# BIT-DYN/OpenObj

Hardware: AMD Instinct MI355X
Metric: training rays/sec/GPU @64 samples/ray, 50 obj; PSNR delta vs ref (higher is better)
Workload: dtype f32; 1 GPU; c2: Replica room_0-shaped, 50 object MLPs on this GPU (hidden 32), 4096 rays/object/step, 64 samples/ray (16+48), RGB+depth+opacity loss, fused fwd+loss+bwd+AdamW; objects_per_gpu=50, objects_total=50, rays_per_object=4096, samples_per_ray=64, hidden=32, feature_head=False, background_mlp=True, parallelism=objects sharded x1, rccl_ranks=1, launched_by=single process, loss_status=0

## Files before the change

include/objnerf_hip.h:

```cpp
#ifndef OBJNERF_HIP_H
#define OBJNERF_HIP_H

#include <stddef.h>
#include <stdint.h>

#ifdef __cplusplus
extern "C" {
#endif

#define OBJNERF_ABI_VERSION 14

#define OBJNERF_OK 0
#define OBJNERF_EINVAL (-22)
#define OBJNERF_ENOTSUP (-95)
#define OBJNERF_ELAUNCH (-5)

#define OBJNERF_N_TENSORS 19

enum objnerf_tensor {
  OBJNERF_T_IN_W = 0, OBJNERF_T_IN_B, OBJNERF_T_M1_W, OBJNERF_T_M1_B, OBJNERF_T_CAT_W,
  OBJNERF_T_CAT_B, OBJNERF_T_M2_W, OBJNERF_T_M2_B, OBJNERF_T_ALPHA_W, OBJNERF_T_ALPHA_B,
  OBJNERF_T_CL_W, OBJNERF_T_CL_B, OBJNERF_T_OC_W, OBJNERF_T_OC_B, OBJNERF_T_FL_W, OBJNERF_T_FL_B,
  OBJNERF_T_OF_W, OBJNERF_T_OF_B, OBJNERF_T_PE_B
};
// ... 46 lines not shown
  float box[4];
} objnerf_ingest_item;
int objnerf_ingest_frame(int32_t W, int32_t H, const uint8_t* rgb, const float* depth, const int32_t* inst,
                         const float* t_wc, int32_t K, const objnerf_ingest_item* items, void* stream);

int objnerf_box_rays(int64_t P, const float* T_WC, const float* T_OC, const float* half_extent,
                     const float* dirs_C, float* out_dirs_W, float* out_near, float* out_far,
                     uint8_t* out_hit, void* stream);
int objnerf_box_points(int64_t n, int32_t n_bins, const float* origin , const float* dirs_W,
                       const float* near, const float* far, const float* u, uint64_t seed, uint32_t draw,
                       float* out_z, float* out_pts, void* stream);

int objnerf_render_fwd(const objnerf_net* net, int64_t n, int32_t n_bins, const float* params, const float* scale,
                       const float* origin , const float* dirs_W, const float* near, const float* far,
                       const float* u, uint64_t seed, uint32_t draw, float* out_depth, float* out_opacity,
                       float* out_rgb, float* out_hfeat, float* out_z, int32_t mode, void* stream);

int objnerf_eval_points(const objnerf_net* net, int32_t K, int64_t N, const float* params,
                        int64_t p_stride, const float* scale, const float* pts, float* out_alpha,
                        float* out_color, float* out_hfeat, float* out_clip, void* stream);

size_t objnerf_eval_workspace_bytes(const objnerf_net* net, int32_t K, int64_t N);
int objnerf_eval_points_ws(const objnerf_net* net, int32_t K, int64_t N, const float* params,
                           int64_t p_stride, const float* scale, const float* pts, float* out_alpha,
                           float* out_color, float* out_hfeat, float* out_clip, void* workspace,
                           size_t workspace_bytes, void* stream);

int objnerf_mlp_forward(const objnerf_net* net, int32_t K, int64_t N, const float* params,
                        int64_t p_stride, const float* emb, float* out_alpha, float* out_color,
                        float* out_hfeat, float* out_clip, void* stream);

int objnerf_mlp_forward_ws(const objnerf_net* net, int32_t K, int64_t N, const float* params,
                           int64_t p_stride, const float* emb, float* out_alpha, float* out_color,
                           float* out_hfeat, float* out_clip, void* workspace, size_t workspace_bytes,
                           void* stream);

size_t objnerf_mlp_backward_workspace_bytes(const objnerf_net* net, int32_t K, int64_t N, int32_t with_clip);
int objnerf_mlp_backward_ws(const objnerf_net* net, int32_t K, int64_t N, const float* params,
                            int64_t p_stride, const float* emb, const float* d_alpha, const float* d_color,
                            const float* d_clip, float* grads, float* d_emb, void* workspace,
                            size_t workspace_bytes, void* stream);

int objnerf_embed_bwd(const objnerf_net* net, int32_t K, int64_t N, const float* params, int64_t p_stride,
                      const float* scale, const float* pts, const float* d_emb, float* d_B, float* scratch,
                      void* stream);

int objnerf_embed(const objnerf_net* net, int32_t K, int64_t N, const float* params,
                  int64_t p_stride, const float* scale, const float* pts, float* out_emb,
                  void* stream);

#define OBJNERF_COMPOSITE_INPUT_IS_OCCUPANCY 1
int objnerf_composite(int64_t n_rays, int32_t S, int32_t flags, const float* alpha, const float* color,
                      const float* z, const float* vals, int32_t V, float* out_term,
                      float* out_depth, float* out_var, float* out_rgb, float* out_opacity,
                      float* out_vals, void* stream);

int objnerf_mfma_peak(int32_t dtype, int32_t iters, int32_t n_wg, float* sink, void* stream);

int objnerf_occupancy(int64_t n, const float* alpha, float* out, void* stream);

int objnerf_feature_head(const objnerf_net* net, int32_t K, int64_t n, const float* params,
                         int64_t p_stride, const float* hfeat, const float* weight, float* out,
                         void* stream);

typedef struct objnerf_loss_args {
  int32_t K, R, S, C;
  float color_scaling, opacity_scaling, feat_scaling, reserved;
  const float* alpha; const float* color; const float* z; const float* gt_depth;
  const float* gt_rgb; const uint8_t* labels; const float* pred_feat; const float* gt_feat;
  const int32_t* flags_in;
  const int32_t* counts_in;
  float* loss_terms; float* total; float* d_alpha; float* d_color; float* d_pred_feat;
  int32_t* counts; int32_t* status;
} objnerf_loss_args;
int objnerf_step_batch_loss(const objnerf_loss_args* a, void* stream);

int objnerf_label_counts(int32_t K, int32_t R, const uint8_t* labels, int32_t* counts,
                         int32_t* flags_out, void* stream);

#define OBJNERF_TRAIN_BF16 1
#define OBJNERF_TRAIN_FP16 4
#define OBJNERF_TRAIN_LAYERWISE 2
#define OBJNERF_TRAIN_SELF_COUNTS 8
struct objnerf_context;
int objnerf_context_create(struct objnerf_context** out);
int objnerf_context_destroy(struct objnerf_context* ctx);

typedef struct objnerf_adamw_args {
  float* exp_avg; float* exp_avg_sq;
  int32_t* group_steps; int32_t bank; int32_t reserved;
  float lr, beta1, beta2, eps, weight_decay, reserved_f;
} objnerf_adamw_args;

typedef struct objnerf_train_args {
  int32_t K, R, S, mode;
  float color_scaling, opacity_scaling, feat_scaling, obj_center;
  const float* params; int64_t p_stride; const float* scale;
  const float* pts; const float* origins; const float* dirs; const float* z;
  const float* gt_depth; const float* gt_rgb; const uint8_t* labels; const float* gt_feat;
  const int32_t* counts; const int32_t* flags;
  float* grads; float* loss_terms; int32_t* status;
  void* workspace; size_t workspace_bytes;
  uint8_t* relu_masks;
  struct objnerf_context* context;
  float* emb_debug;
  const objnerf_adamw_args* optim;
} objnerf_train_args;
size_t objnerf_train_workspace_bytes(const objnerf_net* net, int32_t K, int32_t R, int32_t S,
                                     int32_t with_feat);
int objnerf_train_step(const objnerf_net* net, const objnerf_train_args* a, void* stream);

int objnerf_adamw_step(int32_t K, int64_t P, int64_t p_stride, float* params, const float* grads,
                       float* exp_avg, float* exp_avg_sq, const uint8_t* has_grad, int32_t step,
                       float lr, float beta1, float beta2, float eps, float weight_decay,
                       void* stream);

int objnerf_adamw_step_flags(int32_t K, int64_t P, int64_t p_stride, float* params, const float* grads, float* exp_avg,
                             float* exp_avg_sq, const uint8_t* has_grad, const int32_t* flags, int32_t* group_steps,
                             int32_t bank, int64_t colour_lo, int64_t feature_lo, int64_t feature_hi, float lr,
                             float beta1, float beta2, float eps, float weight_decay, void* stream);

int objnerf_render(int64_t n_rays, int32_t S, int32_t C, const float* termination, const float* vals, float* out,
                   void* stream);

int objnerf_render_loss(int64_t n, int32_t C, int32_t mode, int32_t normalise, const float* render, const float* gt,
                        float* out, void* stream);
int objnerf_reduce_batch_loss(int32_t K, int32_t R, const float* loss_mat, const float* var, const uint8_t* mask,
                              int32_t l2, int32_t avg, int32_t* counts_ws, float* out, int32_t* status, void* stream);
int objnerf_make_grid(int32_t dim, float lo, float hi, const float* scale, const float* transform, float* out,
                      void* stream);
int objnerf_ray_box(int64_t n, const float* origins, const float* dirs, const float* bmin, const float* bmax,
                    float* out_near, float* out_far, uint8_t* out_hit, void* stream);
int objnerf_dirs_w(int64_t F, int64_t P, const float* T_WC, const float* dirs_C, float* out_dirs_W, void* stream);
int objnerf_stratified_bins(int64_t n_rays, int32_t n_bins, const float* lo, float lo_scalar, const float* hi,
                            float hi_scalar, const float* u, uint64_t seed, uint64_t offset, float* out, void* stream);
int objnerf_normal_bins(int64_t n_rays, int32_t n_bins, const float* depth, float delta, const float* g, uint64_t seed,
                        uint64_t offset, float* out, void* stream);

#define OBJNERF_MC_DESCENT 1
size_t objnerf_mc_workspace_bytes(int32_t dim);
int objnerf_mc_count(int32_t dim, float level, const float* vol, void* ws, size_t ws_bytes, int64_t* out_counts,
                     void* stream);
int objnerf_mc_emit(int32_t dim, float level, int32_t flags, const float* vol, void* ws, size_t ws_bytes,
                    int64_t max_verts, int64_t max_faces, float* out_verts, float* out_normals, int32_t* out_faces,
                    void* stream);
int objnerf_mc_tables(uint8_t* edge_c0, uint8_t* edge_axis, uint8_t* ntri, uint8_t* tri);

typedef struct objnerf_voxel_args {
  int32_t K, F, W, H;
  double fx, fy, cx, cy, voxel;
  const objnerf_kf_store* table; const int32_t* n_keyframes; const double* camera_pose;
  const objnerf_kf_crops* crops;
} objnerf_voxel_args;
size_t objnerf_voxel_workspace_bytes(int32_t K, int32_t F, int32_t W, int32_t H);
int objnerf_voxel_scan(const objnerf_voxel_args* a, void* ws, size_t ws_bytes, int64_t* out_total, double* out_minmax,
                       void* stream);
int objnerf_voxel_emit(const objnerf_voxel_args* a, const void* ws, size_t ws_bytes, int32_t k0, int32_t k1,
                       const int64_t* base, const double* vmin, const int64_t* dims, int64_t n_points, double* out_pts,
                       int64_t* out_keys, void* stream);
size_t objnerf_voxel_heads_workspace_bytes(int64_t n);
int objnerf_voxel_heads(int64_t n, const int64_t* sorted_keys, int64_t* ws, void* stream);
int objnerf_voxel_centroids(int64_t n, const int64_t* sorted_keys, const int64_t* perm, const double* pts,
                            const int64_t* ws, int64_t max_voxels, double* out_centroids, int64_t* out_keys,
                            int64_t* out_first, void* stream);

typedef struct objnerf_obb_args {
  int32_t K, reserved;
  const double* verts; const int64_t* vert_off; const double* normals; const int32_t* edges; const int32_t* cand;
  const int64_t* cand_off; const int32_t* mode;
} objnerf_obb_args;
int objnerf_obb_search(const objnerf_obb_args* a, int32_t n_split, double* ws, double* out, void* stream);

#define OBJNERF_PROJ_COSINE 1
#define OBJNERF_PROJ_PER_SEGMENT 2
typedef struct objnerf_project_args {
  int32_t S, D, Q, flags;
  int64_t V, row_stride;
  const float* feat; const int64_t* seg_off; const float* W; const float* bias;
  float* out; float* minmax;
} objnerf_project_args;
size_t objnerf_project_workspace_bytes(int32_t S, int32_t Q, int64_t V);
int objnerf_project(const objnerf_project_args* a, void* ws, size_t ws_bytes, void* stream);

typedef struct objnerf_moments_args {
  int32_t S, D;
  int64_t V, row_stride;
  const float* feat; const int64_t* seg_off;
  double* mean; double* scatter;
} objnerf_moments_args;
size_t objnerf_moments_workspace_bytes(int32_t S, int32_t D);
int objnerf_moments(const objnerf_moments_args* a, void* ws, size_t ws_bytes, void* stream);

#define OBJNERF_COLOR_RGB 0
// ... 222 lines not shown
```

openobj_amd/_lib.py:

```python
from __future__ import annotations

import ctypes as C
import os
from typing import Optional

import torch

_HERE = os.path.dirname(os.path.abspath(__file__))
LIB_PATH = os.environ.get("OBJNERF_LIB") or os.path.join(_HERE, "csrc", "libobjnerf_hip.so")

OBJNERF_N_TENSORS = 19
ABI_VERSION = 14


class ObjnerfError(RuntimeError):
    pass


class Net(C.Structure):
    _fields_ = [("hidden", C.c_int32), ("feat_dim", C.c_int32), ("n_freqs", C.c_int32),
                ("reserved", C.c_int32)]


class SampleArgs(C.Structure):
    _fields_ = [("F", C.c_int32), ("W", C.c_int32), ("H", C.c_int32), ("n_frames", C.c_int32),
                ("n_px", C.c_int32), ("n_cam2surf", C.c_int32), ("n_bins", C.c_int32),
                ("obj_index", C.c_int32),
                ("surface_eps", C.c_float), ("stop_eps", C.c_float), ("min_bound", C.c_float),
                ("obj_center", C.c_float),
                ("rgbs", C.c_void_p), ("depth", C.c_void_p), ("t_wc", C.c_void_p), ("bbox", C.c_void_p),
                ("rays_dir_cache", C.c_void_p),
                ("kf_ids", C.c_void_p), ("u_w", C.c_void_p), ("u_h", C.c_void_p), ("u", C.c_void_p),
                ("g", C.c_void_p),
                ("out_rgb", C.c_void_p), ("out_depth", C.c_void_p), ("out_valid", C.c_void_p),
                ("out_labels", C.c_void_p), ("out_z", C.c_void_p), ("out_pts", C.c_void_p),
                ("max_depth_ws", C.c_void_p),
                ("seed", C.c_uint64), ("draw", C.c_uint32), ("reserved", C.c_uint32),
                ("kf_meta", C.c_void_p), ("out_kf", C.c_void_p), ("out_px", C.c_void_p),
                ("out_origins", C.c_void_p), ("out_dirs", C.c_void_p),
                ("global_partfeat", C.c_void_p), ("use_frame", C.c_void_p), ("out_partfeat", C.c_void_p),
                ("pf_frames", C.c_int32), ("pf_w", C.c_int32), ("pf_h", C.c_int32), ("pf_c", C.c_int32),
                ("pf_stride", C.c_int32), ("part_down", C.c_float),
                ("part_index", C.c_void_p), ("pf_rows", C.c_int32), ("reserved_pf", C.c_int32)]


class IngestItem(C.Structure):
    _fields_ = [("rgbs", C.c_void_p), ("depth", C.c_void_p), ("t_wc", C.c_void_p), ("bbox", C.c_void_p),
                ("slot", C.c_int32), ("obj_id", C.c_int32), ("box", C.c_float * 4)]


class LossArgs(C.Structure):
    _fields_ = [("K", C.c_int32), ("R", C.c_int32), ("S", C.c_int32), ("C", C.c_int32),
                ("color_scaling", C.c_float), ("opacity_scaling", C.c_float),
                ("feat_scaling", C.c_float), ("reserved", C.c_float),
                ("alpha", C.c_void_p), ("color", C.c_void_p), ("z", C.c_void_p), ("gt_depth", C.c_void_p),
                ("gt_rgb", C.c_void_p), ("labels", C.c_void_p), ("pred_feat", C.c_void_p),
                ("gt_feat", C.c_void_p), ("flags_in", C.c_void_p), ("counts_in", C.c_void_p),
                ("loss_terms", C.c_void_p), ("total", C.c_void_p), ("d_alpha", C.c_void_p),
                ("d_color", C.c_void_p), ("d_pred_feat", C.c_void_p),
                ("counts", C.c_void_p), ("status", C.c_void_p)]


TRAIN_BF16 = 1
TRAIN_SELF_COUNTS = 8


class AdamWArgs(C.Structure):
    _fields_ = [("exp_avg", C.c_void_p), ("exp_avg_sq", C.c_void_p), ("group_steps", C.c_void_p),
                ("bank", C.c_int32), ("reserved", C.c_int32),
                ("lr", C.c_float), ("beta1", C.c_float), ("beta2", C.c_float), ("eps", C.c_float),
                ("weight_decay", C.c_float), ("reserved_f", C.c_float)]


class TrainArgs(C.Structure):
    _fields_ = [("K", C.c_int32), ("R", C.c_int32), ("S", C.c_int32), ("mode", C.c_int32),
                ("color_scaling", C.c_float), ("opacity_scaling", C.c_float),
                ("feat_scaling", C.c_float), ("obj_center", C.c_float),
                ("params", C.c_void_p), ("p_stride", C.c_int64), ("scale", C.c_void_p),
                ("pts", C.c_void_p), ("origins", C.c_void_p), ("dirs", C.c_void_p), ("z", C.c_void_p),
                ("gt_depth", C.c_void_p), ("gt_rgb", C.c_void_p), ("labels", C.c_void_p),
                ("gt_feat", C.c_void_p),
                ("counts", C.c_void_p), ("flags", C.c_void_p),
                ("grads", C.c_void_p), ("loss_terms", C.c_void_p), ("status", C.c_void_p),
                ("workspace", C.c_void_p), ("workspace_bytes", C.c_size_t),
                ("relu_masks", C.c_void_p), ("context", C.c_void_p), ("emb_debug", C.c_void_p),
                ("optim", C.c_void_p)]


class KfStore(C.Structure):
    _fields_ = [("rgbs", C.c_void_p), ("depth", C.c_void_p), ("t_wc", C.c_void_p), ("bbox", C.c_void_p)]


class KfCrops(C.Structure):
    _fields_ = [("base", C.c_void_p), ("cap", C.c_int64), ("rect", C.c_void_p), ("t_wc", C.c_void_p),
                ("bbox", C.c_void_p)]


class IngestCropItem(C.Structure):
    _fields_ = [("store", KfCrops), ("slot", C.c_int32), ("obj_id", C.c_int32), ("box", C.c_float * 4),
                ("rect", C.c_int32 * 4)]


class VoxelArgs(C.Structure):
    _fields_ = [("K", C.c_int32), ("F", C.c_int32), ("W", C.c_int32), ("H", C.c_int32),
                ("fx", C.c_double), ("fy", C.c_double), ("cx", C.c_double), ("cy", C.c_double), ("voxel", C.c_double),
                ("table", C.c_void_p), ("n_keyframes", C.c_void_p), ("camera_pose", C.c_void_p),
                ("crops", C.c_void_p)]


class ObbArgs(C.Structure):
    _fields_ = [("K", C.c_int32), ("reserved", C.c_int32), ("verts", C.c_void_p), ("vert_off", C.c_void_p),
                ("normals", C.c_void_p), ("edges", C.c_void_p), ("cand", C.c_void_p), ("cand_off", C.c_void_p),
                ("mode", C.c_void_p)]


class ProjectArgs(C.Structure):
    _fields_ = [("S", C.c_int32), ("D", C.c_int32), ("Q", C.c_int32), ("flags", C.c_int32),
                ("V", C.c_int64), ("row_stride", C.c_int64),
                ("feat", C.c_void_p), ("seg_off", C.c_void_p), ("W", C.c_void_p), ("bias", C.c_void_p),
                ("out", C.c_void_p), ("minmax", C.c_void_p)]


class MomentsArgs(C.Structure):
    _fields_ = [("S", C.c_int32), ("D", C.c_int32), ("V", C.c_int64), ("row_stride", C.c_int64),
                ("feat", C.c_void_p), ("seg_off", C.c_void_p), ("mean", C.c_void_p), ("scatter", C.c_void_p)]


class ColorArgs(C.Structure):
    _fields_ = [("S", C.c_int32), ("Q", C.c_int32), ("V", C.c_int64), ("rgb_stride", C.c_int64),
                ("seg_off", C.c_void_p), ("mode", C.c_void_p), ("rgb", C.c_void_p), ("factor", C.c_void_p),
                ("constant", C.c_void_p), ("column", C.c_void_p), ("proj", C.c_void_p), ("minmax", C.c_void_p),
                ("out", C.c_void_p)]


class RayBoxesArgs(C.Structure):
    _fields_ = [("F", C.c_int32), ("N", C.c_int32), ("W", C.c_int32), ("H", C.c_int32),
                ("fx", C.c_double), ("fy", C.c_double), ("cx", C.c_double), ("cy", C.c_double),
                ("depth", C.c_void_p), ("twc", C.c_void_p), ("boxes", C.c_void_p), ("out", C.c_void_p)]


class MaskPointsArgs(C.Structure):
    _fields_ = [("n", C.c_int64), ("W", C.c_int32), ("H", C.c_int32),
                ("fx", C.c_double), ("fy", C.c_double), ("cx", C.c_double), ("cy", C.c_double),
                ("pix", C.c_void_p), ("depth", C.c_void_p), ("pose", C.c_void_p), ("out", C.c_void_p)]


class MapPointsHead(C.Structure):
# ... 5 lines not shown
    _fields_ = [("of_w", C.c_void_p), ("of_b", C.c_void_p), ("hfeat", C.c_void_p), ("row0", C.c_int64),
                ("n_rows", C.c_int64), ("H", C.c_int32), ("reserved", C.c_int32)]


class AffinityArgs(C.Structure):
    _fields_ = [("N", C.c_int32), ("F", C.c_int32), ("d_cap", C.c_int32), ("d_clip", C.c_int32),
                ("w_geo", C.c_double), ("w_cap", C.c_double), ("w_clip", C.c_double), ("w_color", C.c_double),
                ("w_geo2d", C.c_double),
                ("boxes", C.c_void_p), ("cap", C.c_void_p), ("clip", C.c_void_p), ("color", C.c_void_p),
                ("boxes2d", C.c_void_p), ("W", C.c_void_p), ("terms", C.c_void_p)]


PROJ_COSINE = 1
PROJ_PER_SEGMENT = 2
COLOR_RGB, COLOR_CONSTANT, COLOR_RAINBOW, COLOR_PCA = 0, 1, 2, 3


SIGNATURES = {
    "objnerf_abi_version": (C.c_int, []),
    "objnerf_context_create": (C.c_int, [C.POINTER(C.c_void_p)]),
    "objnerf_context_destroy": (C.c_int, [C.c_void_p]),
    "objnerf_param_layout": (C.c_int64, [C.POINTER(Net), C.POINTER(C.c_int64)]),
    "objnerf_rays_dirs": (C.c_int, [C.c_int32, C.c_int32, C.c_float, C.c_float, C.c_float, C.c_float,
                                    C.c_void_p, C.c_void_p]),
    "objnerf_sample_rays": (C.c_int, [C.POINTER(SampleArgs), C.c_void_p]),
    "objnerf_sample_rays_stacked": (C.c_int, [C.POINTER(SampleArgs), C.c_int32, C.c_void_p, C.c_void_p]),
    "objnerf_sample_points": (C.c_int, [C.POINTER(SampleArgs), C.c_void_p, C.c_void_p, C.c_void_p, C.c_void_p, C.c_void_p]),
    "objnerf_ingest_frame": (C.c_int, [C.c_int32, C.c_int32, C.c_void_p, C.c_void_p, C.c_void_p, C.c_void_p, C.c_int32,
                                       C.c_void_p, C.c_void_p]),
    "objnerf_box_rays": (C.c_int, [C.c_int64, C.c_void_p, C.c_void_p, C.c_void_p, C.c_void_p, C.c_void_p, C.c_void_p,
                                   C.c_void_p, C.c_void_p, C.c_void_p]),
    "objnerf_box_points": (C.c_int, [C.c_int64, C.c_int32, C.c_void_p, C.c_void_p, C.c_void_p, C.c_void_p, C.c_void_p,
                                     C.c_uint64, C.c_uint32, C.c_void_p, C.c_void_p, C.c_void_p]),
    "objnerf_render_fwd": (C.c_int, [C.POINTER(Net), C.c_int64, C.c_int32, C.c_void_p, C.c_void_p, C.c_void_p, C.c_void_p,
                                     C.c_void_p, C.c_void_p, C.c_void_p, C.c_uint64, C.c_uint32, C.c_void_p, C.c_void_p,
                                     C.c_void_p, C.c_void_p, C.c_void_p, C.c_int32, C.c_void_p]),
    "objnerf_eval_points": (C.c_int, [C.POINTER(Net), C.c_int32, C.c_int64, C.c_void_p, C.c_int64,
                                      C.c_void_p, C.c_void_p, C.c_void_p, C.c_void_p, C.c_void_p,
                                      C.c_void_p, C.c_void_p]),
    "objnerf_eval_workspace_bytes": (C.c_size_t, [C.POINTER(Net), C.c_int32, C.c_int64]),
    "objnerf_eval_points_ws": (C.c_int, [C.POINTER(Net), C.c_int32, C.c_int64, C.c_void_p, C.c_int64,
                                         C.c_void_p, C.c_void_p, C.c_void_p, C.c_void_p, C.c_void_p,
                                         C.c_void_p, C.c_void_p, C.c_size_t, C.c_void_p]),
    "objnerf_mlp_forward": (C.c_int, [C.POINTER(Net), C.c_int32, C.c_int64, C.c_void_p, C.c_int64,
                                      C.c_void_p, C.c_void_p, C.c_void_p, C.c_void_p, C.c_void_p,
                                      C.c_void_p]),
    "objnerf_mlp_forward_ws": (C.c_int, [C.POINTER(Net), C.c_int32, C.c_int64, C.c_void_p, C.c_int64,
                                         C.c_void_p, C.c_void_p, C.c_void_p, C.c_void_p, C.c_void_p,
                                         C.c_void_p, C.c_size_t, C.c_void_p]),
    "objnerf_embed": (C.c_int, [C.POINTER(Net), C.c_int32, C.c_int64, C.c_void_p, C.c_int64, C.c_void_p,
                                C.c_void_p, C.c_void_p, C.c_void_p]),
    "objnerf_mlp_backward_workspace_bytes": (C.c_size_t, [C.POINTER(Net), C.c_int32, C.c_int64, C.c_int32]),
    "objnerf_mlp_backward_ws": (C.c_int, [C.POINTER(Net), C.c_int32, C.c_int64, C.c_void_p, C.c_int64, C.c_void_p,
                                          C.c_void_p, C.c_void_p, C.c_void_p, C.c_void_p, C.c_void_p, C.c_void_p,
                                          C.c_size_t, C.c_void_p]),
    "objnerf_embed_bwd": (C.c_int, [C.POINTER(Net), C.c_int32, C.c_int64, C.c_void_p, C.c_int64, C.c_void_p, C.c_void_p,
                                    C.c_void_p, C.c_void_p, C.c_void_p, C.c_void_p]),
    "objnerf_occupancy": (C.c_int, [C.c_int64, C.c_void_p, C.c_void_p, C.c_void_p]),
    "objnerf_render": (C.c_int, [C.c_int64, C.c_int32, C.c_int32, C.c_void_p, C.c_void_p, C.c_void_p, C.c_void_p]),
    "objnerf_render_loss": (C.c_int, [C.c_int64, C.c_int32, C.c_int32, C.c_int32, C.c_void_p, C.c_void_p, C.c_void_p,
                                      C.c_void_p]),
    "objnerf_reduce_batch_loss": (C.c_int, [C.c_int32, C.c_int32, C.c_void_p, C.c_void_p, C.c_void_p, C.c_int32, C.c_int32,
                                            C.c_void_p, C.c_void_p, C.c_void_p, C.c_void_p]),
    "objnerf_make_grid": (C.c_int, [C.c_int32, C.c_float, C.c_float, C.c_void_p, C.c_void_p, C.c_void_p, C.c_void_p]),
    "objnerf_ray_box": (C.c_int, [C.c_int64, C.c_void_p, C.c_void_p, C.c_void_p, C.c_void_p, C.c_void_p, C.c_void_p,
                                  C.c_void_p, C.c_void_p]),
    "objnerf_dirs_w": (C.c_int, [C.c_int64, C.c_int64, C.c_void_p, C.c_void_p, C.c_void_p, C.c_void_p]),
    "objnerf_stratified_bins": (C.c_int, [C.c_int64, C.c_int32, C.c_void_p, C.c_float, C.c_void_p, C.c_float, C.c_void_p,
                                          C.c_uint64, C.c_uint64, C.c_void_p, C.c_void_p]),
    "objnerf_normal_bins": (C.c_int, [C.c_int64, C.c_int32, C.c_void_p, C.c_float, C.c_void_p, C.c_uint64, C.c_uint64,
                                      C.c_void_p, C.c_void_p]),
    "objnerf_mfma_peak": (C.c_int, [C.c_int32, C.c_int32, C.c_int32, C.c_void_p, C.c_void_p]),
    "objnerf_composite": (C.c_int, [C.c_int64, C.c_int32, C.c_int32, C.c_void_p, C.c_void_p, C.c_void_p, C.c_void_p,
                                    C.c_int32, C.c_void_p, C.c_void_p, C.c_void_p, C.c_void_p, C.c_void_p,
                                    C.c_void_p, C.c_void_p]),
    "objnerf_feature_head": (C.c_int, [C.POINTER(Net), C.c_int32, C.c_int64, C.c_void_p, C.c_int64,
                                       C.c_void_p, C.c_void_p, C.c_void_p, C.c_void_p]),
    "objnerf_step_batch_loss": (C.c_int, [C.POINTER(LossArgs), C.c_void_p]),
    "objnerf_label_counts": (C.c_int, [C.c_int32, C.c_int32, C.c_void_p, C.c_void_p, C.c_void_p,
                                       C.c_void_p]),
    "objnerf_train_workspace_bytes": (C.c_size_t, [C.POINTER(Net), C.c_int32, C.c_int32, C.c_int32,
                                                   C.c_int32]),
    "objnerf_train_step": (C.c_int, [C.POINTER(Net), C.POINTER(TrainArgs), C.c_void_p]),
    "objnerf_adamw_step": (C.c_int, [C.c_int32, C.c_int64, C.c_int64, C.c_void_p, C.c_void_p, C.c_void_p,
                                     C.c_void_p, C.c_void_p, C.c_int32, C.c_float, C.c_float, C.c_float,
                                     C.c_float, C.c_float, C.c_void_p]),
    "objnerf_adamw_step_flags": (C.c_int, [C.c_int32, C.c_int64, C.c_int64, C.c_void_p, C.c_void_p, C.c_void_p, C.c_void_p,
                                           C.c_void_p, C.c_void_p, C.c_void_p, C.c_int32, C.c_int64, C.c_int64, C.c_int64,
                                           C.c_float, C.c_float, C.c_float, C.c_float, C.c_float, C.c_void_p]),
    "objnerf_mc_workspace_bytes": (C.c_size_t, [C.c_int32]),
    "objnerf_mc_count": (C.c_int, [C.c_int32, C.c_float, C.c_void_p, C.c_void_p, C.c_size_t, C.c_void_p, C.c_void_p]),
    "objnerf_mc_emit": (C.c_int, [C.c_int32, C.c_float, C.c_int32, C.c_void_p, C.c_void_p, C.c_size_t, C.c_int64,
                                  C.c_int64, C.c_void_p, C.c_void_p, C.c_void_p, C.c_void_p]),
    "objnerf_mc_tables": (C.c_int, [C.c_void_p, C.c_void_p, C.c_void_p, C.c_void_p]),
    "objnerf_voxel_workspace_bytes": (C.c_size_t, [C.c_int32, C.c_int32, C.c_int32, C.c_int32]),
    "objnerf_voxel_scan": (C.c_int, [C.POINTER(VoxelArgs), C.c_void_p, C.c_size_t, C.c_void_p, C.c_void_p, C.c_void_p]),
    "objnerf_voxel_emit": (C.c_int, [C.POINTER(VoxelArgs), C.c_void_p, C.c_size_t, C.c_int32, C.c_int32, C.c_void_p,
                                     C.c_void_p, C.c_void_p, C.c_int64, C.c_void_p, C.c_void_p, C.c_void_p]),
    "objnerf_voxel_heads_workspace_bytes": (C.c_size_t, [C.c_int64]),
    "objnerf_voxel_heads": (C.c_int, [C.c_int64, C.c_void_p, C.c_void_p, C.c_void_p]),
    "objnerf_voxel_centroids": (C.c_int, [C.c_int64, C.c_void_p, C.c_void_p, C.c_void_p, C.c_void_p, C.c_int64,
                                          C.c_void_p, C.c_void_p, C.c_void_p, C.c_void_p]),
    "objnerf_obb_search": (C.c_int, [C.POINTER(ObbArgs), C.c_int32, C.c_void_p, C.c_void_p, C.c_void_p]),
    "objnerf_project_workspace_bytes": (C.c_size_t, [C.c_int32, C.c_int32, C.c_int64]),
    "objnerf_project": (C.c_int, [C.POINTER(ProjectArgs), C.c_void_p, C.c_size_t, C.c_void_p]),
    "objnerf_moments_workspace_bytes": (C.c_size_t, [C.c_int32, C.c_int32]),
    "objnerf_moments": (C.c_int, [C.POINTER(MomentsArgs), C.c_void_p, C.c_size_t, C.c_void_p]),
    "objnerf_vertex_colors": (C.c_int, [C.POINTER(ColorArgs), C.c_void_p]),
    "objnerf_rainbow_lut": (C.c_int, [C.c_void_p]),
    "objnerf_cell_keys": (C.c_int, [C.c_int64, C.c_int32, C.c_void_p, C.c_void_p, C.c_double, C.c_double, C.c_void_p,
                                    C.c_void_p, C.c_void_p, C.c_void_p]),
    "objnerf_dbscan_workspace_bytes": (C.c_size_t, [C.c_int64]),
    "objnerf_dbscan": (C.c_int, [C.c_int64, C.c_int32, C.c_void_p, C.c_void_p, C.c_void_p, C.c_void_p, C.c_void_p,
                                 C.c_double, C.c_void_p, C.c_size_t, C.c_void_p, C.c_void_p]),
    "objnerf_cloud_overlap": (C.c_int, [C.c_int64, C.c_int32, C.c_void_p, C.c_void_p, C.c_void_p, C.c_void_p, C.c_double,
                                        C.c_void_p, C.c_void_p]),
    "objnerf_mask_ray_boxes": (C.c_int, [C.POINTER(RayBoxesArgs), C.c_void_p]),
    "objnerf_mask_points": (C.c_int, [C.POINTER(MaskPointsArgs), C.c_void_p]),
    "objnerf_mask_hist": (C.c_int, [C.c_int64, C.c_int32, C.c_void_p, C.c_void_p, C.c_void_p, C.c_int32, C.c_int32,
                                    C.c_void_p, C.c_void_p]),
    "objnerf_point_bounds": (C.c_int, [C.c_int64, C.c_int32, C.c_void_p, C.c_void_p, C.c_void_p, C.c_void_p]),
    "objnerf_affinity_workspace_bytes": (C.c_size_t, [C.c_int32]),
    "objnerf_mask_affinity": (C.c_int, [C.POINTER(AffinityArgs), C.c_void_p, C.c_size_t, C.c_void_p, C.c_void_p]),
    "objnerf_mask_edges": (C.c_int, [C.c_int32, C.c_void_p, C.c_void_p, C.c_int64, C.c_void_p, C.c_void_p, C.c_void_p]),
    "objnerf_part_index": (C.c_int, [C.c_int32, C.c_int32, C.c_int32, C.c_void_p, C.c_void_p, C.c_void_p]),
    "objnerf_part_dense": (C.c_int, [C.c_int64, C.c_int32, C.c_int32, C.c_void_p, C.c_void_p, C.c_void_p, C.c_void_p]),
    "objnerf_ingest_frame_crops": (C.c_int, [C.c_int32, C.c_int32, C.c_void_p, C.c_void_p, C.c_void_p, C.c_void_p,
                                             C.c_int32, C.c_void_p, C.c_void_p, C.c_void_p]),
    "objnerf_sample_rays_crops": (C.c_int, [C.POINTER(SampleArgs), C.c_int32, C.c_void_p, C.c_void_p]),
    "objnerf_mappoints_workspace_bytes": (C.c_size_t, [C.c_int64, C.c_int32]),
    "objnerf_mappoints_count": (C.c_int, [C.c_int64, C.c_int32, C.c_void_p, C.c_void_p, C.c_void_p, C.c_size_t, C.c_void_p,
                                          C.c_void_p]),
    "objnerf_mappoints_emit": (C.c_int, [C.c_int64, C.c_int32, C.c_void_p, C.c_void_p, C.c_void_p, C.c_size_t, C.c_int64,
                                         C.c_void_p, C.c_void_p]),
    "objnerf_mappoints_eval": (C.c_int, [C.POINTER(Net), C.c_int32, C.c_int64, C.c_int64, C.c_void_p, C.c_int64, C.c_void_p,
                                         C.c_void_p, C.c_void_p, C.c_void_p, C.c_void_p, C.c_void_p, C.c_void_p, C.c_void_p,
                                         C.c_void_p, C.c_void_p, C.c_void_p]),
    "objnerf_mappoints_gather": (C.c_int, [C.c_int64, C.c_void_p, C.c_void_p, C.c_float, C.c_void_p, C.c_void_p]),
    "objnerf_mappoints_merge": (C.c_int, [C.c_int64, C.c_int64, C.c_void_p, C.c_void_p, C.c_int32, C.c_void_p, C.c_void_p]),
    "objnerf_mappoints_resolve": (C.c_int, [C.c_int64, C.c_int32, C.c_int64, C.c_void_p, C.c_void_p, C.c_void_p, C.c_void_p, C.c_void_p,
                                            C.c_void_p, C.c_void_p, C.c_void_p]),
    "objnerf_mappoints_head_workspace_bytes": (C.c_size_t, [C.c_int64]),
    "objnerf_mappoints_head": (C.c_int, [C.c_int32, C.c_int32, C.c_int64, C.c_int64, C.c_void_p, C.c_void_p, C.c_void_p,
                                         C.c_void_p, C.c_int32, C.c_void_p, C.c_size_t, C.c_void_p, C.c_void_p, C.c_void_p]),
    "objnerf_mesh_sample_workspace_bytes": (C.c_size_t, [C.c_int64, C.c_int32]),
    "objnerf_mesh_sample": (C.c_int, [C.c_int64, C.c_int64, C.c_int32, C.c_int64, C.c_void_p, C.c_void_p, C.c_void_p,
                                      C.c_void_p, C.c_uint64, C.c_void_p, C.c_size_t, C.c_void_p, C.c_void_p, C.c_void_p,
                                      C.c_void_p]),
    "objnerf_nearest_workspace_bytes": (C.c_size_t, [C.c_int64, C.c_int32]),
    "objnerf_nearest": (C.c_int, [C.c_int64, C.c_int64, C.c_int32, C.c_void_p, C.c_void_p, C.c_void_p, C.c_void_p,
                                  C.c_void_p, C.c_double, C.c_void_p, C.c_void_p, C.c_int32, C.c_void_p, C.c_size_t,
                                  C.c_void_p, C.c_void_p, C.c_void_p, C.c_void_p]),
    "objnerf_seg_stats": (C.c_int, [C.c_int64, C.c_int32, C.c_void_p, C.c_void_p, C.c_int32, C.POINTER(C.c_double),
                                    C.c_void_p, C.c_void_p]),
    "objnerf_vertex_views": (C.c_int, [C.c_int64, C.c_int32, C.c_int32, C.c_int32, C.c_void_p, C.c_void_p, C.c_void_p,
                                       C.c_double, C.c_double, C.c_double, C.c_double, C.c_double, C.c_double, C.c_int32,
                                       C.c_void_p, C.c_void_p]),
    "objnerf_mesh_cull_workspace_bytes": (C.c_size_t, [C.c_int64, C.c_int64]),
    "objnerf_mesh_cull_count": (C.c_int, [C.c_int64, C.c_int64, C.c_int32, C.c_void_p, C.c_void_p, C.c_void_p, C.c_size_t,
                                          C.c_void_p, C.c_void_p, C.c_void_p]),
    "objnerf_mesh_cull_emit": (C.c_int, [C.c_int64, C.c_int64, C.c_int32, C.c_void_p, C.c_void_p, C.c_void_p, C.c_size_t,
                                         C.c_int64, C.c_int64, C.c_void_p, C.c_void_p, C.c_void_p, C.c_void_p, C.c_void_p]),
    "objnerf_view_rays_workspace_bytes": (C.c_size_t, [C.c_int64, C.c_int32]),
    "objnerf_view_rays_count": (C.c_int, [C.c_int64, C.c_int32, C.c_void_p, C.c_void_p, C.c_void_p, C.c_void_p, C.c_size_t,
                                          C.c_void_p, C.c_void_p]),
    "objnerf_view_rays_emit": (C.c_int, [C.c_int64, C.c_int32, C.c_void_p, C.c_void_p, C.c_void_p, C.c_void_p, C.c_size_t,
# ... 102 lines not shown
```

openobj_amd/csrc/objnerf_generic.h:

```cpp
#pragma once
#include "../../include/objnerf_hip.h"
namespace objmisc {
struct LossHoisted {
  int Hh;
  const float* hf; const float* rayin; const float* gram;
  float* d_hf; float* rayfeat;
};
int step_batch_loss_impl(const objnerf_loss_args* a, const LossHoisted* hz, void* stream, float* loss_part);
int adamw_flags_range(int32_t K, int64_t P, int64_t p_stride, float* params, const float* grads, float* exp_avg,
                      float* exp_avg_sq, const uint8_t* has_grad, const int32_t* flags, int32_t* group_steps, int32_t bank,
                      int64_t colour_lo, int64_t feature_lo, int64_t feature_hi, int64_t ng_lo, int64_t ng_hi, float lr,
                      float beta1, float beta2, float eps, float weight_decay, void* stream);
int label_counts_only(int32_t K, int32_t R, const uint8_t* labels, int32_t* counts, void* stream);
}

namespace objgen {
size_t train_workspace_bytes(const objnerf_net* net, int K, int R, int S, int feat, int sixteen = 0);
int train_step(const objnerf_net* net, const objnerf_train_args* a, void* stream, int* done = nullptr);
struct Operand { const float* p; long s0, s1, bs; bool h16; };
inline Operand op_rows(const float* p, long ld, long bs, bool h16 = false) { return {p, ld, 1, bs, h16}; }
inline Operand op_cols(const float* p, long ld, long bs, bool h16 = false) { return {p, 1, ld, bs, h16}; }
struct FeatHeadArgs { int K, R, Hh, C; const float* P; long ps; int off_w, off_b; const float* gt_feat; };
void feat_gram(void* stream, const FeatHeadArgs& h, float* gram, long gstride);
void feature_head(void* stream, const FeatHeadArgs& h, long n, const float* hfeat, const float* weight, float* out);
void gemm_f32(void* stream, int batch, int M, int N, int Kd, const Operand& A, const Operand& B, const Operand& C,
              bool accumulate);
size_t wgrad_parts_floats(int batch, int M, int N, long n);
void wgrad_f32(void* stream, int batch, int M, int N, long n, const Operand& A, const Operand& B, const Operand& C,
               float* parts, size_t parts_floats);
struct FeatHead {
  float *gram, *rayin, *rayfeat, *X1, *X2, *Tm, *mom, *parts; size_t parts_floats;
};
size_t feat_head_workspace_bytes(int K, int R, int Hh, int C);
FeatHead feat_head_carve(char* base, int K, int R, int Hh, int C);
int feat_head_prep(void* stream, const FeatHeadArgs& h, const FeatHead& f, int operands);
int feat_head_grads(void* stream, const FeatHeadArgs& h, const FeatHead& f, float* grads, int operands);
size_t eval_workspace_bytes(const objnerf_net* net, int K, long N);
int eval_points(const objnerf_net* net, int K, long N, const float* params, long p_stride, const float* scale,
                const float* pts, float* out_alpha, float* out_color, float* out_hfeat, float* out_clip,
                void* workspace, size_t workspace_bytes, void* stream, const float* emb_in = nullptr);
size_t mlp_backward_workspace_bytes(const objnerf_net* net, int K, long N, int with_clip);
int mlp_backward(const objnerf_net* net, int K, long N, const float* params, long p_stride, const float* emb,
                 const float* d_alpha, const float* d_color, const float* d_clip, float* grads, float* d_emb,
                 void* workspace, size_t workspace_bytes, void* stream);
int embed_backward(const objnerf_net* net, int K, long N, const float* params, long p_stride, const float* scale,
                   const float* pts, const float* d_emb, float* d_B, float* scratch, void* stream);
}

namespace obj256 {
bool applicable(const objnerf_net* net, const objnerf_train_args* a);
size_t workspace_bytes(int K, int R, int S, int feat = 0, int C = 0);
int train_step(const objnerf_net* net, const objnerf_train_args* a, void* stream);
}
```

openobj_amd/csrc/objnerf_misc.hip:

```cpp
#include "objnerf_device.h"
#include "objnerf_philox.h"
#include "objnerf_wg.h"
#include "objnerf_generic.h"
#include "objnerf_step_tail.h"
#include "objnerf_boxray.h"

namespace {

__device__ __forceinline__ float sgnf(float x) { return x > 0.f ? 1.0f : (x < 0.f ? -1.0f : 0.0f); }

__global__ __launch_bounds__(256) void composite_kernel(long n_rays, int S, int in_is_occ, const float* alpha,
                                                        const float* color, const float* z, const float* vals,
                                                        int V, float* out_term,
                                                        float* out_depth, float* out_var, float* out_rgb,
                                                        float* out_opacity, float* out_vals) {
  extern __shared__ float sm[];
  const int lane = threadIdx.x & 63, w = threadIdx.x >> 6;
  float* wv = sm + (long)w * S;
  const long ray = (long)blockIdx.x * 4 + w;
  if (ray >= n_rays) return;
  float carry = 1.0f, D = 0.f, O = 0.f, C0 = 0.f, C1 = 0.f, C2 = 0.f;
  for (int s0 = 0; s0 < S; s0 += 64) {
    const int s = s0 + lane;
    const bool on = s < S;
    const float al = on ? alpha[ray * S + s] : 0.f;
    const float occ = on ? (in_is_occ ? al : sigmoid_acc(al)) : 0.f;
    const float fr = on ? (1.0f - occ) + 1e-10f : 1.0f;
    const float pinc = SegRows::make(64, lane).scan_mul(fr, lane) * carry;
    float T = __shfl_up(pinc, 1, 64);
    if (lane == 0) T = carry;
    carry = __shfl(pinc, 63, 64);
    const float wt = occ * T;
    if (on) {
      wv[s] = wt;
      if (out_term) out_term[ray * S + s] = wt;
    }
    const float zz = (on && z) ? z[ray * S + s] : 0.f;
    D += wave_sum64(wt * zz);
    O += wave_sum64(wt);
    if (color) {
      const float* cp = color + (ray * S + s) * 3;
      C0 += wave_sum64(on ? wt * cp[0] : 0.f);
      C1 += wave_sum64(on ? wt * cp[1] : 0.f);
      C2 += wave_sum64(on ? wt * cp[2] : 0.f);
    }
  }
  float Vv = 0.f;
  for (int s0 = 0; s0 < S; s0 += 64) {
    const int s = s0 + lane;
    const bool on = s < S;
    const float dz = (on && z) ? z[ray * S + s] - D : 0.f;
    Vv += wave_sum64(on ? wv[s] * (dz * dz) : 0.f);
  }
  if (lane == 0) {
    if (out_depth) out_depth[ray] = D;
    if (out_var) out_var[ray] = Vv;
    if (out_opacity) out_opacity[ray] = O;
    if (out_rgb) { out_rgb[ray * 3] = C0; out_rgb[ray * 3 + 1] = C1; out_rgb[ray * 3 + 2] = C2; }
  }
  if (vals && out_vals) {
    for (int v = lane; v < V; v += 64) {
      float acc = 0.f;
      for (int s = 0; s < S; ++s) acc += wv[s] * vals[(ray * S + s) * (long)V + v];
      out_vals[ray * (long)V + v] = acc;
    }
  }
}


__global__ void embed_kernel(int K, long N, int n_freqs, const float* params, long p_stride, long off_B,
                             const float* scale, const float* pts, float* out) {
  const int E = 3 + OBJ_NDIR * n_freqs;
  const long idx = (long)blockIdx.x * blockDim.x + threadIdx.x;
  const int k = blockIdx.y;
  if (idx >= N * E) return;
  const long i = idx / E;
  const int e = (int)(idx - i * E);
  const float* B = params + (long)k * p_stride + off_B;
  const float sc = scale[k];
  const float* p = pts + ((long)k * N + i) * 3;
  float v;
  if (e < 3) {
    v = p[e] / sc;
  } else {
    const float t0 = p[0] / sc, t1 = p[1] / sc, t2 = p[2] / sc;
    const int f = (e - 3) / OBJ_NDIR, j = (e - 3) - f * OBJ_NDIR;
    const float pj = fmaf(t2, B[3 * j + 2], fmaf(t1, B[3 * j + 1], t0 * B[3 * j]));
    v = sin_acc((pj * (float)(1 << f)) * OBJ_PI_F);
  }
  out[(long)k * N * E + idx] = v;
}

__global__ void occupancy_kernel(long n, const float* alpha, float* out) {
  const long i = (long)blockIdx.x * blockDim.x + threadIdx.x;
  if (i < n) out[i] = sigmoid_acc(alpha[i]);
}

__global__ void label_counts_kernel(int K, int R, const uint8_t* labels, int* counts, int* flags) {
  const int k = blockIdx.x;
  int c1 = 0, c2 = 0;
  for (int r = threadIdx.x; r < R; r += blockDim.x) {
    const int l = labels[(long)k * R + r];
    c1 += (l == 1);
    c2 += (l != 2);
  }
  __shared__ int s1[4], s2[4];
  for (int d = 32; d >= 1; d >>= 1) {
    c1 += __shfl_xor(c1, d, 64);
    c2 += __shfl_xor(c2, d, 64);
  }
  if ((threadIdx.x & 63) == 0) { s1[threadIdx.x >> 6] = c1; s2[threadIdx.x >> 6] = c2; }
  __syncthreads();
  if (threadIdx.x == 0) {
    const int a = s1[0] + s1[1] + s1[2] + s1[3], b = s2[0] + s2[1] + s2[2] + s2[3];
    counts[2 * k] = a;
    counts[2 * k + 1] = b;
    if (!flags) return;
    if (K == 1) {
      flags[0] = a == 0;
      flags[1] = b == 0;
    } else {
      if (a == 0) atomicOr(&flags[0], 1);
      if (b == 0) atomicOr(&flags[1], 1);
    }
  }
}

__global__ void loss_prologue_kernel(int K, const int* counts_in, int* counts, int* flags, const int* flags_in,
                                     float* loss_terms) {
  __shared__ int f[2];
  if (threadIdx.x < 2) f[threadIdx.x] = (flags_in && flags_in[threadIdx.x]) ? 1 : 0;
  __syncthreads();
  for (int k = threadIdx.x; k < K; k += blockDim.x) {
    const int a = counts_in[2 * k], b = counts_in[2 * k + 1];
    counts[2 * k] = a;
    counts[2 * k + 1] = b;
    if (a == 0) atomicOr(&f[0], 1);
    if (b == 0) atomicOr(&f[1], 1);
  }
  for (int i = threadIdx.x; i < 4 * K; i += blockDim.x) loss_terms[i] = 0.f;
  __syncthreads();
  if (threadIdx.x < 2) flags[threadIdx.x] = f[threadIdx.x];
}

__global__ void merge_flags_kernel(int* flags, const int* flags_in) {
  if (threadIdx.x < 2 && flags_in && flags_in[threadIdx.x]) flags[threadIdx.x] = 1;
}

struct LossDev {
  int K, R, S, C;
  float cs, os, fs;
  const float* alpha; const float* color; const float* z; const float* gt_depth; const float* gt_rgb;
  const uint8_t* labels; const float* pred_feat; const float* gt_feat;
  const int* counts; const int* flags;
  float* loss_terms; float* d_alpha; float* d_color; float* d_pred_feat;
  int Hh;
  const float* hf;
  const float* rayin;
  const float* gram;
  float* d_hf;
  float* rayfeat;
  float* loss_part;
};

__global__ __launch_bounds__(1024) void loss_kernel(const LossDev a) {
  extern __shared__ float sm[];
  __shared__ float s_red[16][4];
  const int lane = threadIdx.x & 63, w = threadIdx.x >> 6;
  const int nw = blockDim.x >> 6;
  const int S = a.S;
  float* wv = sm + (long)w * (3 * S + 2 * a.Hh);
  float* tv = wv + S;
  float* dwv = tv + S;
  float* sfh = dwv + S;
  float* sgf = sfh + a.Hh;
  const long rr = (long)blockIdx.x * nw + w;
  const int k = (int)(rr / a.R);
  const float n1 = (float)a.counts[2 * k], n2 = (float)a.counts[2 * k + 1];
  const float inv1 = a.flags[0] ? 0.0f : 1.0f / (n1 + 1e-10f);
  const float inv2 = a.flags[1] ? 0.0f : 1.0f / (n2 + 1e-10f);
  const int lab = a.labels[rr];
  const float m1 = (lab == 1) ? 1.f : 0.f, m2 = (lab != 2) ? 1.f : 0.f, tgt = (lab != 0) ? 1.f : 0.f;
  float carry = 1.0f, D = 0.f, O = 0.f, C0 = 0.f, C1 = 0.f, C2 = 0.f;
  for (int s0 = 0; s0 < S; s0 += 64) {
    const int s = s0 + lane;
    const bool on = s < S;
    const float occ = on ? sigmoid_acc(a.alpha[rr * S + s]) : 0.f;
    const float fr = on ? (1.0f - occ) + 1e-10f : 1.0f;
    const float pinc = SegRows::make(64, lane).scan_mul(fr, lane) * carry;
    float T = __shfl_up(pinc, 1, 64);
    if (lane == 0) T = carry;
    carry = __shfl(pinc, 63, 64);
    const float wt = occ * T;
    if (on) { wv[s] = wt; tv[s] = T; dwv[s] = 0.f; }
    const float* cp = a.color + (rr * S + (on ? s : 0)) * 3;
    D += wave_sum64(on ? wt * a.z[rr * S + s] : 0.f);
    O += wave_sum64(wt);
    C0 += wave_sum64(on ? wt * cp[0] : 0.f);
    C1 += wave_sum64(on ? wt * cp[1] : 0.f);
    C2 += wave_sum64(on ? wt * cp[2] : 0.f);
  }
  float Vv = 0.f;
  for (int s0 = 0; s0 < S; s0 += 64) {
    const int s = s0 + lane;
    const bool on = s < S;
    const float dz = on ? a.z[rr * S + s] - D : 0.f;
// ... 494 lines not shown
  const float* o = origins_ws + (long)i * 3;
  const float* dr = dirs_ws + (long)i * 3;
  for (int s = 0; s < S; ++s) {
    float* p = a.out_pts + ((long)i * S + s) * 3;
    p[0] = (o[0] + dr[0] * z[s]) - a.obj_center;
    p[1] = (o[1] + dr[1] * z[s]) - a.obj_center;
    p[2] = (o[2] + dr[2] * z[s]) - a.obj_center;
  }
}

__global__ void sample_prepare_kernel(const objnerf_sample_args a, const uint8_t* __restrict__ rgbs4,
                                      const float* __restrict__ depth, const float* __restrict__ origins,
                                      const float* __restrict__ dirs_w, float* origins_ws, float* dirs_ws) {
  const int i = blockIdx.x * blockDim.x + threadIdx.x;
  const int n = a.n_frames * a.n_px;
  if (i >= n) return;
  const uint8_t* px = rgbs4 + (long)i * 4;
  a.out_rgb[i * 3] = px[0]; a.out_rgb[i * 3 + 1] = px[1]; a.out_rgb[i * 3 + 2] = px[2];
  a.out_labels[i] = px[3];
  const float d = depth[i];
  a.out_depth[i] = d;
  atomicMax((int*)a.max_depth_ws, __float_as_int(fmaxf(d, 0.0f)));
  const int f = i / a.n_px;
#pragma unroll
  for (int r = 0; r < 3; ++r) {
    origins_ws[i * 3 + r] = origins[f * 3 + r];
    dirs_ws[i * 3 + r] = dirs_w[i * 3 + r];
  }
}

}

#define CLEAR_STALE() (void)hipGetLastError()

namespace objmisc {
int step_batch_loss_impl(const objnerf_loss_args* a, const LossHoisted* hz, void* stream, float* loss_part) {
  CLEAR_STALE();
  if (!a || !a->alpha || !a->color || !a->z || !a->gt_depth || !a->gt_rgb || !a->labels || !a->loss_terms ||
      !a->counts || a->K <= 0 || a->R <= 0 || a->S <= 0)
    return OBJNERF_EINVAL;
  if (!hz && (a->pred_feat == nullptr) != (a->gt_feat == nullptr)) return OBJNERF_EINVAL;
  if (hz && (!a->gt_feat || a->pred_feat || !hz->hf || !hz->rayin || !hz->gram || !hz->d_hf || !hz->rayfeat || hz->Hh <= 0))
    return OBJNERF_EINVAL;
  if (a->S > 2048) return OBJNERF_ENOTSUP;
  hipStream_t st = (hipStream_t)stream;
  int* flags = a->counts + 2 * a->K;
  if (a->counts_in) {
    hipLaunchKernelGGL(loss_prologue_kernel, dim3(1), dim3(256), 0, st, a->K, a->counts_in, a->counts, flags, a->flags_in,
                       a->loss_terms);
  } else {
    if (a->K > 1) (void)hipMemsetAsync(flags, 0, 2 * sizeof(int), st);
    hipLaunchKernelGGL(label_counts_kernel, dim3(a->K), dim3(256), 0, st, a->K, a->R, a->labels, a->counts, flags);
    if (a->flags_in) hipLaunchKernelGGL(merge_flags_kernel, dim3(1), dim3(64), 0, st, flags, a->flags_in);
    (void)hipMemsetAsync(a->loss_terms, 0, (size_t)a->K * 4 * sizeof(float), st);
  }
  LossDev d;
  d.K = a->K; d.R = a->R; d.S = a->S; d.C = a->C;
  d.cs = a->color_scaling; d.os = a->opacity_scaling; d.fs = a->feat_scaling;
  d.alpha = a->alpha; d.color = a->color; d.z = a->z; d.gt_depth = a->gt_depth; d.gt_rgb = a->gt_rgb;
  d.labels = a->labels; d.pred_feat = a->pred_feat; d.gt_feat = a->gt_feat; d.counts = a->counts; d.flags = flags;
  d.loss_terms = a->loss_terms; d.d_alpha = a->d_alpha; d.d_color = a->d_color; d.d_pred_feat = a->d_pred_feat;
  d.Hh = hz ? hz->Hh : 0;
  d.hf = hz ? hz->hf : nullptr; d.rayin = hz ? hz->rayin : nullptr; d.gram = hz ? hz->gram : nullptr;
  d.d_hf = hz ? hz->d_hf : nullptr; d.rayfeat = hz ? hz->rayfeat : nullptr;
  const long nr = (long)a->K * a->R;
  int rb = 16;
  while (rb > 1 && (a->R % rb != 0 || (size_t)rb * (3 * a->S + 2 * d.Hh) * 4 > 60000)) rb >>= 1;
  d.loss_part = loss_part;
  hipLaunchKernelGGL(loss_kernel, dim3((unsigned)(nr / rb)), dim3(64 * rb), (size_t)rb * (3 * a->S + 2 * d.Hh) * 4, st, d);
  CHECK_LAUNCH();
  hipLaunchKernelGGL(loss_total_kernel, dim3(1), dim3(256), 0, st, a->K, a->loss_terms, a->color_scaling,
                     a->opacity_scaling, (a->pred_feat || hz) ? a->feat_scaling : 0.0f, a->total, a->status,
                     (const float*)loss_part, a->R / rb);
  CHECK_LAUNCH();
  return OBJNERF_OK;
}
int label_counts_only(int32_t K, int32_t R, const uint8_t* labels, int32_t* counts, void* stream) {
  CLEAR_STALE();
  if (K <= 0 || R <= 0 || !labels || !counts) return OBJNERF_EINVAL;
  hipLaunchKernelGGL(label_counts_kernel, dim3(K), dim3(256), 0, (hipStream_t)stream, K, R, labels, counts, (int*)nullptr);
  CHECK_LAUNCH();
  return OBJNERF_OK;
}
int adamw_flags_range(int32_t K, int64_t P, int64_t p_stride, float* params, const float* grads, float* exp_avg,
                      float* exp_avg_sq, const uint8_t* has_grad, const int32_t* flags, int32_t* group_steps, int32_t bank,
                      int64_t colour_lo, int64_t feature_lo, int64_t feature_hi, int64_t ng_lo, int64_t ng_hi, float lr,
                      float beta1, float beta2, float eps, float weight_decay, void* stream) {
  CLEAR_STALE();
  if (K <= 0 || P <= 0 || p_stride < P || !params || !grads || !exp_avg || !exp_avg_sq || !flags || !group_steps ||
      (bank != 0 && bank != 1) ||
      colour_lo > feature_lo || feature_lo > feature_hi || feature_hi > P)
    return OBJNERF_EINVAL;
  dim3 grid((unsigned)((P + 255) / 256), (unsigned)K);
  hipLaunchKernelGGL(adamw_dyn_kernel, grid, dim3(256), 0, (hipStream_t)stream, (long)P, (long)p_stride, params, grads,
                     exp_avg, exp_avg_sq, has_grad, flags, group_steps, (int)bank, (long)colour_lo, (long)feature_lo,
                     (long)feature_hi, (double)lr, (double)beta1, (double)beta2, eps, (double)weight_decay, (long)ng_lo,
                     (long)ng_hi);
  CHECK_LAUNCH();
  return OBJNERF_OK;
}
}

template <int DT>
__global__ __launch_bounds__(256) void mfma_peak_kernel(int iters, float* sink) {
  typedef float f16v __attribute__((ext_vector_type(16)));
  typedef __bf16 bf8 __attribute__((ext_vector_type(8)));
  const int lane = threadIdx.x & 63;
  f16v a0, a1;
  for (int i = 0; i < 16; ++i) { a0[i] = 0.f; a1[i] = 0.f; }
  const float av = 0.37f + 0.011f * lane, bv = -0.52f + 0.007f * (lane ^ 21);
  bf8 ab, bb;
  for (int i = 0; i < 8; ++i) { ab[i] = (__bf16)(av + 0.05f * i); bb[i] = (__bf16)(bv - 0.03f * i); }
  for (int i = 0; i < iters; ++i) {
    if (DT == 0) {
      a0 = __builtin_amdgcn_mfma_f32_32x32x2f32(av, bv, a0, 0, 0, 0);
      a1 = __builtin_amdgcn_mfma_f32_32x32x2f32(bv, av, a1, 0, 0, 0);
      a0 = __builtin_amdgcn_mfma_f32_32x32x2f32(av, av, a0, 0, 0, 0);
      a1 = __builtin_amdgcn_mfma_f32_32x32x2f32(bv, bv, a1, 0, 0, 0);
    } else {
      a0 = __builtin_amdgcn_mfma_f32_32x32x16_bf16(ab, bb, a0, 0, 0, 0);
      a1 = __builtin_amdgcn_mfma_f32_32x32x16_bf16(bb, ab, a1, 0, 0, 0);
      a0 = __builtin_amdgcn_mfma_f32_32x32x16_bf16(ab, ab, a0, 0, 0, 0);
      a1 = __builtin_amdgcn_mfma_f32_32x32x16_bf16(bb, bb, a1, 0, 0, 0);
    }
    if ((i & 127) == 127) { a0 *= 1e-3f; a1 *= 1e-3f; }
  }
  float r = 0.f;
  for (int i = 0; i < 16; ++i) r += a0[i] + a1[i];
  sink[blockIdx.x * 256 + threadIdx.x] = r;
}

extern "C" {

int objnerf_composite(int64_t n_rays, int32_t S, int32_t flags, const float* alpha, const float* color,
                      const float* z, const float* vals, int32_t V, float* out_term, float* out_depth, float* out_var,
                      float* out_rgb, float* out_opacity, float* out_vals, void* stream) {
  CLEAR_STALE();
  if (n_rays <= 0 || S <= 0 || !alpha) return OBJNERF_EINVAL;
  if (!z && (out_depth || out_var)) return OBJNERF_EINVAL;
  if (S > 4096) return OBJNERF_ENOTSUP;
  hipLaunchKernelGGL(composite_kernel, dim3((unsigned)((n_rays + 3) / 4)), dim3(256), (size_t)4 * S * 4,
                     (hipStream_t)stream, (long)n_rays, S, (int)(flags & OBJNERF_COMPOSITE_INPUT_IS_OCCUPANCY), alpha,
                     color, z, vals, V, out_term, out_depth, out_var, out_rgb, out_opacity, out_vals);
  CHECK_LAUNCH();
  return OBJNERF_OK;
}

int objnerf_mfma_peak(int32_t dtype, int32_t iters, int32_t n_wg, float* sink, void* stream) {
  CLEAR_STALE();
  if (!sink || iters <= 0 || n_wg <= 0 || (dtype != 0 && dtype != 1)) return OBJNERF_EINVAL;
  if (dtype == 0) hipLaunchKernelGGL(mfma_peak_kernel<0>, dim3(n_wg), dim3(256), 0, (hipStream_t)stream, iters, sink);
  else hipLaunchKernelGGL(mfma_peak_kernel<1>, dim3(n_wg), dim3(256), 0, (hipStream_t)stream, iters, sink);
  CHECK_LAUNCH();
  return OBJNERF_OK;
}

int objnerf_occupancy(int64_t n, const float* alpha, float* out, void* stream) {
  CLEAR_STALE();
  if (n <= 0 || !alpha || !out) return OBJNERF_EINVAL;
  hipLaunchKernelGGL(occupancy_kernel, dim3((unsigned)((n + 255) / 256)), dim3(256), 0, (hipStream_t)stream, (long)n,
                     alpha, out);
  CHECK_LAUNCH();
  return OBJNERF_OK;
}

int objnerf_feature_head(const objnerf_net* net, int32_t K, int64_t n, const float* params, int64_t p_stride,
// ... 207 lines not shown
```

openobj_amd/csrc/objnerf_train.hip:

```cpp
#include <mutex>
#include "objnerf_mlp32.h"
#include "objnerf_train_common.h"
#include "objnerf_generic.h"
#include "objnerf_wg.h"
#include "objnerf_step_tail.h"

using namespace obj32;
using namespace objtrain;

namespace {

struct EvalDev {
  int K, G; long N;
  const float* params; long p_stride; const float* scale; const float* pts; const float* emb;
  float* alpha; float* color; float* hfeat;
  Layout L;
};

constexpr int XCOLS = 33;
struct FinalizeArgs {
  const float* slab; const float* loss_part;
  int K, G; long P, slab_stride, p_stride;
  long ng_lo, ng_hi, ext_lo, ext_hi;
  float* grads; float* loss_terms; int* status;
  int flat_nwg, NT, Gs;
  float* params; float* m; float* v; const int* flags; int* steps; int bank;
  long lo1, lo2, hi2;
  double lr, b1, b2, wd; float eps;
  const int* counts_in; int* flags_out;
  const float* Tpart; const float* Mpart; const float* head_w; int Gfin, C; long of_w, of_b;
};
constexpr int FIN_EPT = 4;
__global__ __launch_bounds__(256) void finalize_kernel(const FinalizeArgs a) {
  const int k = blockIdx.y;
  const long i0 = (long)blockIdx.x * (256 * FIN_EPT) + threadIdx.x;
  __shared__ float s_step_size[3], s_bc2_sqrt[3];
  __shared__ int s_active[3];
  __shared__ int s_bad;
  __shared__ float s_M[XCOLS * XCOLS];
  const bool first = blockIdx.x == 0 && blockIdx.y == 0;
  if (a.counts_in && first && threadIdx.x == 64) {
    int e0, e1;
    early_flags_of_counts(a.counts_in, a.K, e0, e1);
    a.flags_out[0] = e0; a.flags_out[1] = e1;
  }
  if (a.params && threadIdx.x < 3) {
    const int g = threadIdx.x;
    int e0, e1;
    if (a.counts_in) early_flags_of_counts(a.counts_in, a.K, e0, e1);
    else { e0 = a.flags[0]; e1 = a.flags[1]; }
    adamw_group_begin(g, e0 != 0, e1 != 0, a.steps, a.bank, a.lr, a.b1, a.b2, first, s_active[g], s_step_size[g],
                      s_bc2_sqrt[g]);
  }
  if (first && threadIdx.x == 0) s_bad = 0;
  const long blk_lo = (long)blockIdx.x * (256 * FIN_EPT), blk_hi = blk_lo + 256 * FIN_EPT;
  const bool head_blk = a.Tpart && blk_lo < a.ext_hi && blk_hi > a.ext_lo;
  if (head_blk)
    for (int e = threadIdx.x; e < XCOLS * XCOLS; e += 256) {
      float v = 0.f;
      for (int g = 0; g < a.Gfin; ++g) v += a.Mpart[((long)k * a.Gfin + g) * XCOLS * XCOLS + e];
      s_M[e] = v;
    }
  if (a.params || first || head_blk) __syncthreads();
  int G = a.G;
  if (a.flat_nwg) {
    const long T = (long)a.K * a.NT;
    G = flat_wg_of(T, a.flat_nwg, (long)(k + 1) * a.NT - 1) - flat_wg_of(T, a.flat_nwg, (long)k * a.NT) + 1;
  }
  const int stride = a.flat_nwg ? a.Gs : a.G;
  float s[FIN_EPT];
  bool live[FIN_EPT], slabbed[FIN_EPT];
#pragma unroll
  for (int e = 0; e < FIN_EPT; ++e) {
    const long i = i0 + 256 * e;
    live[e] = i < a.P && !(i >= a.ng_lo && i < a.ng_hi);
    slabbed[e] = live[e] && !(i >= a.ext_lo && i < a.ext_hi);
    s[e] = 0.f;
  }
  const float* sl0 = a.slab + (long)k * stride * a.slab_stride + i0;
  for (int g = 0; g < G; ++g) {
    float t[FIN_EPT];
#pragma unroll
    for (int e = 0; e < FIN_EPT; ++e) t[e] = slabbed[e] ? sl0[(long)g * a.slab_stride + 256 * e] : 0.f;
#pragma unroll
    for (int e = 0; e < FIN_EPT; ++e) s[e] += t[e];
  }
#pragma unroll
  for (int e = 0; e < FIN_EPT; ++e) {
    const long i = i0 + 256 * e;
    if (!live[e]) continue;
    const long idx = (long)k * a.p_stride + i;
    float sv_ = s[e];
    if (!slabbed[e]) {
      if (a.Tpart) {
        const bool is_b = i >= a.of_b;
        const int cc = is_b ? (int)(i - a.of_b) : (int)((i - a.of_w) >> 5), hh = is_b ? 32 : (int)((i - a.of_w) & 31);
        const float* hw = a.head_w + (long)k * ((long)a.C * 33);
        const float* W = hw + cc * 32;
        const float bc = hw[a.C * 32 + cc];
        float v = 0.f;
        for (int g = 0; g < a.Gfin; ++g) v += a.Tpart[((long)k * a.Gfin + g) * a.C * XCOLS + cc * XCOLS + hh];
        if (!is_b) {
          for (int j = 0; j < 32; ++j) v = fmaf(W[j], s_M[j * XCOLS + hh], v);
          sv_ = fmaf(bc, s_M[32 * XCOLS + hh], v);
        } else {
          for (int j = 0; j < 32; ++j) v = fmaf(W[j], s_M[32 * XCOLS + j], v);
          sv_ = fmaf(bc, s_M[32 * XCOLS + 32], v);
        }
      } else {
        sv_ = a.grads[idx];
      }
    }
    s[e] = sv_;
  }
#pragma unroll
  for (int e = 0; e < FIN_EPT; ++e) {
    const long i = i0 + 256 * e;
    if (!live[e]) continue;
    const long idx = (long)k * a.p_stride + i;
    const float sv_ = s[e];
    if (slabbed[e] || a.Tpart) a.grads[idx] = sv_;
    if (a.params) {
      const int g = adamw_group_of(i, a.lo1, a.lo2, a.hi2);
      if (s_active[g]) {
        float decay, w1, beta2, w2;
        adamw_coeffs(a.lr, a.b1, a.b2, a.wd, decay, w1, beta2, w2);
        adamw_update(a.params, a.m, a.v, idx, sv_, decay, w1, beta2, w2, s_step_size[g], s_bc2_sqrt[g], a.eps);
      }
    }
  }
  if (first) {
    int bad = 0;
    for (int e = threadIdx.x; e < 4 * a.K; e += blockDim.x) {
      const int kk = e >> 2;
      int Gk = a.G;
      if (a.flat_nwg) {
        const long T = (long)a.K * a.NT;
        Gk = flat_wg_of(T, a.flat_nwg, (long)(kk + 1) * a.NT - 1) - flat_wg_of(T, a.flat_nwg, (long)kk * a.NT) + 1;
      }
      float sl = 0.f;
      for (int g = 0; g < Gk; ++g) sl += a.loss_part[((long)kk * stride + g) * 4 + (e & 3)];
      a.loss_terms[e] = sl;
      bad |= loss_status_bits(sl);
    }
    if (bad) atomicOr(&s_bad, bad);
    __syncthreads();
    if (threadIdx.x == 0) *a.status = s_bad;
  }
}

template <bool FEAT, bool FROM_EMB>
__global__ __launch_bounds__(256) void eval_kernel(const EvalDev a) {
  using namespace obj32n;
  extern __shared__ __attribute__((aligned(16))) float lds[];
  const int tid = threadIdx.x, lane = tid & 63;
  const int w = __builtin_amdgcn_readfirstlane(tid >> 6);
  const int c = lane & 15, g = lane >> 4;
  const int k = blockIdx.x / a.G, gi = blockIdx.x % a.G;
  stage_weights32(lds, a.params + (long)k * a.p_stride, a.L, FEAT, tid, 256);
  const float* sv = lds + sv_base(FEAT);
  const float* wf = (const float*)__builtin_assume_aligned(lds + 4 * g * WROW + out_pos(c), 8);
  const float scale = FROM_EMB ? 1.0f : a.scale[k];
  const long ntiles = (a.N + 63) / 64;
  for (long tile = gi; tile < ntiles; tile += a.G) {
    asm volatile("" ::: "memory");
    const long n = tile * 64 + 16 * w + c;
    const bool valid = n < a.N;
    const long o = (long)k * a.N + (valid ? n : 0);
    Emb32 e;
    if (FROM_EMB) {
      embed32_load(e, a.emb + o * OBJ_EMB, g);
    } else {
      const float* p = a.pts + o * 3;
      Pe32 pe;
      pe32_project(sv, g, p[0], p[1], p[2], scale, pe);
      embed32(e, pe, g);
    }
    Acts act;
    const float hout = mlp32_forward<FEAT>(wf, sv, g, e, act);
    if (valid) {
      if (g == 0) a.alpha[o] = hout;
      else a.color[o * 3 + g - 1] = hout;
      if (FEAT) {
#pragma unroll
        for (int tt = 0; tt < 2; ++tt) {
          float4 v = make_float4(act.hf.t[tt][0], act.hf.t[tt][1], act.hf.t[tt][2], act.hf.t[tt][3]);
          *reinterpret_cast<float4*>(a.hfeat + o * H + 16 * tt + 4 * g) = v;
        }
      }
    }
  }
}

__global__ __launch_bounds__(256) void feat_rowstats_kernel(const float* params, long p_stride, int off_b, int C, int R,
                                                            const float* gt_feat, float* rayin) {
  const int k = blockIdx.y;
  const int l16 = threadIdx.x & 15;
  const long r = (long)blockIdx.x * 16 + (threadIdx.x >> 4);
  const float* B = params + (long)k * p_stride + off_b;
  float bs = 0.f, gs = 0.f;
  if (r < R) {
    const float* gp = gt_feat + ((long)k * R + r) * C;
    for (int cc = 4 * l16; cc < C; cc += 64) {
      const float4 gv = *reinterpret_cast<const float4*>(gp + cc);
      bs = fmaf(B[cc + 3], gv.w, fmaf(B[cc + 2], gv.z, fmaf(B[cc + 1], gv.y, fmaf(B[cc], gv.x, bs))));
      gs = fmaf(gv.w, gv.w, fmaf(gv.z, gv.z, fmaf(gv.y, gv.y, fmaf(gv.x, gv.x, gs))));
    }
  }
  bs = dpp_rowsum16(bs);
  gs = dpp_rowsum16(gs);
  if (r < R && l16 == 0) {
    float* o = rayin + ((long)k * R + r) * RAYIN;
    o[32] = bs;
    o[33] = sqrtf(gs);
  }
}
constexpr int FEAT_PRE_MAXC = 512;
__global__ __launch_bounds__(512, 4) void feat_pre_kernel(const float* __restrict__ params, long p_stride, int off_w, int off_b,
                                                       int C, int R, const float* __restrict__ gt_feat,
                                                       float* __restrict__ rayin, float* __restrict__ gram,
                                                       float* __restrict__ head_snap, const uint8_t* __restrict__ labels,
                                                       int* __restrict__ counts) {
  extern __shared__ __attribute__((aligned(16))) float fp_lds[];
  const int k = blockIdx.y, tid = threadIdx.x, lane = tid & 63, w = tid >> 6;
// ... 272 lines not shown
                const float* scale, const float* pts, const float* emb, float* out_alpha, float* out_color,
                float* out_hfeat, float* out_clip, void* stream) {
  EvalDev d;
  d.K = K; d.N = N; d.params = params; d.p_stride = p_stride; d.scale = scale; d.pts = pts; d.emb = emb;
  d.alpha = out_alpha; d.color = out_color; d.hfeat = out_hfeat;
  d.L = make_layout(net->feat_dim);
  const long ntiles = (N + 63) / 64;
  long G = (2L * objnerf_num_cu()) / K;
  if (G < 1) G = 1;
  if (G > ntiles) G = ntiles;
  d.G = (int)G;
  hipStream_t st = (hipStream_t)stream;
  const bool feat = out_hfeat != nullptr;
  const size_t lds_bytes = (size_t)obj32n::img_floats(feat) * 4;
  objnerf_once_per_device([] {
    (void)hipFuncSetAttribute((const void*)eval_kernel<true, true>, hipFuncAttributeMaxDynamicSharedMemorySize,
                              obj32n::img_floats(true) * 4);
    (void)hipFuncSetAttribute((const void*)eval_kernel<true, false>, hipFuncAttributeMaxDynamicSharedMemorySize,
                              obj32n::img_floats(true) * 4);
  });
  const dim3 grid(K * d.G), blk(256);
  if (emb) {
    if (feat) hipLaunchKernelGGL((eval_kernel<true, true>), grid, blk, lds_bytes, st, d);
    else hipLaunchKernelGGL((eval_kernel<false, true>), grid, blk, lds_bytes, st, d);
  } else {
    if (feat) hipLaunchKernelGGL((eval_kernel<true, false>), grid, blk, lds_bytes, st, d);
    else hipLaunchKernelGGL((eval_kernel<false, false>), grid, blk, lds_bytes, st, d);
  }
  if (hipGetLastError() != hipSuccess) return OBJNERF_ELAUNCH;
  if (out_clip) return objnerf_feature_head(net, K, N, params, p_stride, out_hfeat, nullptr, out_clip, stream);
  return OBJNERF_OK;
}

}

extern "C" {

int objnerf_abi_version(void) { return OBJNERF_ABI_VERSION; }

int64_t objnerf_param_layout(const objnerf_net* net, int64_t offsets[OBJNERF_N_TENSORS + 1]) {
  if (!net || !offsets || net->hidden <= 0 || net->feat_dim <= 0) return OBJNERF_EINVAL;
  const int64_t H_ = net->hidden, C = net->feat_dim;
  const int64_t sizes[OBJNERF_N_TENSORS] = {H_ * OBJ_E1, H_, H_ * H_, H_, H_ * (H_ + OBJ_E1), H_, H_ * H_, H_, H_, 1,
                                            H_ * (H_ + OBJ_E2), H_, 3 * H_, 3, H_ * (H_ + OBJ_E2), H_, C * H_, C,
                                            OBJ_NDIR * 3};
  int64_t o = 0;
  for (int i = 0; i < OBJNERF_N_TENSORS; ++i) { offsets[i] = o; o += sizes[i]; }
  offsets[OBJNERF_N_TENSORS] = o;
  return (o + 63) / 64 * 64;
}

static int grid_cap(int K) {
  const int g = objnerf_num_cu() / (K > 0 ? K : 1);
  return g > 32 ? g : 32;
}
static int train_grid(int K, int NT) {
  constexpr long TILE_EQUIV = 4;
  const int cu = objnerf_num_cu();
  int gmax = grid_cap(K);
  if (gmax > NT) gmax = NT;
  if (gmax < 1) gmax = 1;
  int best = 1;
  long best_cost = -1;
  for (int G = 1; G <= gmax; ++G) {
    const long rounds = ((long)K * G + cu - 1) / cu;
    const long cost = rounds * ((NT + G - 1) / G + TILE_EQUIV);
    if (best_cost < 0 || cost < best_cost) { best = G; best_cost = cost; }
  }
  return best;
}

static void choose_flat(TrainDev& d, int K, const long TILE_EQUIV) {
  const int cu = objnerf_num_cu();
  const long T = (long)K * d.NT;
  if (T < cu) return;
  const long share = (T + cu - 1) / cu;
  const long segs = 1 + (share + d.NT - 1) / d.NT;
  const long cost_flat = share + segs * TILE_EQUIV;
  const long rounds = ((long)K * d.G + cu - 1) / cu;
  const long cost_strided = rounds * ((d.NT + d.G - 1) / d.G + TILE_EQUIV);
  const long gs = ((long)d.NT * cu + T - 1) / T + 1;
  if (cost_flat < cost_strided && gs <= grid_cap(K)) { d.flat_nwg = cu; d.Gs = (int)gs; }
}

struct Workspace32 {
  float* slab;
  float* loss_part;
  float *rayin, *gram, *rayfeat;
  float *X1, *X2;
  float *Tm, *mom;
  float *parts_t, *parts_m;
  float* head_snap;
  size_t bytes;
};
static Workspace32 workspace32(uintptr_t base, int K, int R, int C, int64_t ps, bool feat) {
  Workspace32 w = {};
  auto take = [&](size_t floats) { float* p = (float*)(base + w.bytes); w.bytes += align256(floats * 4); return p; };
  w.slab = take((size_t)K * grid_cap(K) * ps);
  w.loss_part = take((size_t)K * grid_cap(K) * 4);
  if (feat) {
    w.rayin = take((size_t)K * R * RAYIN);
    w.gram = take((size_t)K * GRAM);
    w.rayfeat = take((size_t)K * R * RAYFEAT);
    w.X1 = take((size_t)K * R * XCOLS);
    w.X2 = take((size_t)K * R * XCOLS);
    w.Tm = take((size_t)K * C * XCOLS + (size_t)K * XCOLS * XCOLS);
    w.mom = w.Tm + (size_t)K * C * XCOLS;
    w.parts_t = take(objgen::wgrad_parts_floats(K, C, XCOLS, R));
    w.parts_m = take(objgen::wgrad_parts_floats(K, XCOLS, XCOLS, R));
    w.head_snap = take((size_t)K * C * XCOLS);
  }
  return w;
}

size_t objnerf_train_workspace_bytes(const objnerf_net* net, int32_t K, int32_t R, int32_t S, int32_t with_feat) {
  if (!net || K <= 0 || R <= 0 || S <= 0) return 0;
  if (net->hidden != 32 || S > 64 || (with_feat & 2)) return objgen::train_workspace_bytes(net, K, R, S, with_feat & 1, (with_feat & 4) != 0);
  int64_t offs[OBJNERF_N_TENSORS + 1];
  const int64_t ps = objnerf_param_layout(net, offs);
  return workspace32(0, K, R, net->feat_dim, ps, (with_feat & 1) != 0).bytes;
}

int objnerf_train_step(const objnerf_net* net, const objnerf_train_args* a, void* stream) {
  (void)hipGetLastError();
  if (!net || !a || !a->params || !a->scale || !a->z || !a->gt_depth || !a->gt_rgb || !a->labels || !a->counts ||
      !a->flags || !a->grads || !a->loss_terms || !a->status || !a->workspace)
    return OBJNERF_EINVAL;
  if (!a->pts && (!a->origins || !a->dirs)) return OBJNERF_EINVAL;
  if (a->K <= 0 || a->R <= 0 || a->S <= 0) return OBJNERF_EINVAL;
  if (net->n_freqs != 6) return OBJNERF_ENOTSUP;
  if ((a->mode & OBJNERF_TRAIN_FP16) && (a->mode & OBJNERF_TRAIN_BF16)) return OBJNERF_EINVAL;
  if (a->optim && (!a->optim->exp_avg || !a->optim->exp_avg_sq || !a->optim->group_steps ||
                   (a->optim->bank != 0 && a->optim->bank != 1)))
    return OBJNERF_EINVAL;
  if (net->hidden != 32 || a->S > 64 || (a->mode & (OBJNERF_TRAIN_LAYERWISE | OBJNERF_TRAIN_FP16))) {
    if (a->workspace_bytes < objgen::train_workspace_bytes(net, a->K, a->R, a->S, a->gt_feat != nullptr,
                                                           (a->mode & (OBJNERF_TRAIN_FP16 | OBJNERF_TRAIN_BF16)) != 0))
      return OBJNERF_EINVAL;
    if (a->emb_debug) return OBJNERF_ENOTSUP;
    int done = 0;
    int rc;
#ifndef OBJ_NO_TRAIN256
    if (!(a->mode & OBJNERF_TRAIN_LAYERWISE) && obj256::applicable(net, a)) {
      if (a->mode & OBJNERF_TRAIN_SELF_COUNTS) {
        rc = objnerf_label_counts(a->K, a->R, a->labels, const_cast<int32_t*>(a->counts), const_cast<int32_t*>(a->flags), stream);
        if (rc) return rc;
      }
      rc = obj256::train_step(net, a, stream);
    } else
#endif
    rc = objgen::train_step(net, a, stream, &done);
    if (rc) return rc;
    if (a->optim && !(done & 2)) {
      int64_t offs[OBJNERF_N_TENSORS + 1];
      objnerf_param_layout(net, offs);
      const bool feat_ = a->gt_feat != nullptr;
      const objnerf_adamw_args* o = a->optim;
      return objmisc::adamw_flags_range(a->K, offs[OBJNERF_N_TENSORS], a->p_stride, const_cast<float*>(a->params), a->grads,
                                        o->exp_avg, o->exp_avg_sq, nullptr, a->flags, o->group_steps, o->bank,
                                        offs[OBJNERF_T_CL_W], offs[OBJNERF_T_FL_W], offs[OBJNERF_T_PE_B],
                                        feat_ ? offs[OBJNERF_N_TENSORS] : offs[OBJNERF_T_FL_W],
                                        feat_ ? offs[OBJNERF_N_TENSORS] : offs[OBJNERF_T_PE_B], o->lr, o->beta1, o->beta2,
                                        o->eps, o->weight_decay, stream);
    }
    return OBJNERF_OK;
  }
  const bool self_counts = (a->mode & OBJNERF_TRAIN_SELF_COUNTS) != 0;
  const bool feat = a->gt_feat != nullptr;
  const bool counts_in_pre = self_counts && feat && net->feat_dim <= FEAT_PRE_MAXC && net->feat_dim % 16 == 0;
  if (self_counts && !counts_in_pre) {
    const int rc = objmisc::label_counts_only(a->K, a->R, a->labels, const_cast<int32_t*>(a->counts), stream);
    if (rc) return rc;
  }
  if (feat && (TS / a->S) > 16) return OBJNERF_ENOTSUP;
  const bool bf16 = (a->mode & OBJNERF_TRAIN_BF16) != 0;
  if (bf16 && (a->relu_masks || a->emb_debug)) return OBJNERF_ENOTSUP;
  int64_t offs[OBJNERF_N_TENSORS + 1];
  const int64_t ps = objnerf_param_layout(net, offs);
  if (a->p_stride < offs[OBJNERF_N_TENSORS]) return OBJNERF_EINVAL;
  const int C = net->feat_dim;
  const Workspace32 ws = workspace32((uintptr_t)a->workspace, a->K, a->R, C, ps, feat);
  if (a->workspace_bytes < ws.bytes) return OBJNERF_EINVAL;

  TrainDev d;
  d.K = a->K; d.R = a->R; d.S = a->S;
  d.TR = TS / a->S;
  d.NT = (a->R + d.TR - 1) / d.TR;
  d.G = train_grid(a->K, d.NT);
  d.flat_nwg = 0; d.Gs = 0;
  d.color_scaling = a->color_scaling; d.opacity_scaling = a->opacity_scaling; d.feat_scaling = a->feat_scaling;
  d.obj_center = a->obj_center;
  d.params = a->params; d.p_stride = a->p_stride; d.scale = a->scale;
  d.pts = a->pts; d.origins = a->origins; d.dirs = a->dirs; d.z = a->z;
  d.gt_depth = a->gt_depth; d.gt_rgb = a->gt_rgb; d.labels = a->labels; d.gt_feat = a->gt_feat;
  d.counts = a->counts; d.flags = a->flags; d.derive_flags = self_counts ? 1 : 0;
  d.L = make_layout(net->feat_dim);
  d.slab = ws.slab;
  d.slab_stride = ps;
  d.loss_part = ws.loss_part;
  d.rayin = ws.rayin; d.gram = ws.gram; d.rayfeat = ws.rayfeat;
  d.relu_masks = a->relu_masks;
  d.emb_debug = a->emb_debug;

  hipStream_t st = (hipStream_t)stream;
  const float *fin_T = nullptr, *fin_M = nullptr;
  int fin_G = 0;
  if (feat) {
    const bool pre_one = C <= FEAT_PRE_MAXC && C % 16 == 0;
    if (!pre_one) objgen::feat_gram(stream, {a->K, 0, 32, C, a->params, (long)a->p_stride, d.L.of_w, d.L.of_b, nullptr}, ws.gram, GRAM);
    if (pre_one) {
      const size_t pre_lds = ((size_t)(C / 16) * 2 * 64 * 4 + C) * sizeof(float);
      objnerf_once_per_device([] {
        (void)hipFuncSetAttribute((const void*)feat_pre_kernel, hipFuncAttributeMaxDynamicSharedMemorySize,
                                  (int)(((FEAT_PRE_MAXC / 16) * 2 * 64 * 4 + FEAT_PRE_MAXC) * sizeof(float)));
      });
      int gpo = 2 * objnerf_num_cu() / a->K;
      if (gpo < 1) gpo = 1;
      if (gpo > (a->R + 127) / 128) gpo = (a->R + 127) / 128;
      hipLaunchKernelGGL(feat_pre_kernel, dim3(gpo, a->K), dim3(512), pre_lds, st, a->params, (long)a->p_stride,
                         d.L.of_w, d.L.of_b, C, a->R, a->gt_feat, ws.rayin, ws.gram, ws.head_snap, a->labels,
                         counts_in_pre ? const_cast<int32_t*>(a->counts) : nullptr);
    } else {
      objgen::gemm_f32(stream, a->K, a->R, 32, C, objgen::op_rows(a->gt_feat, C, (long)a->R * C),
                       objgen::op_rows(a->params + d.L.of_w, 32, (long)a->p_stride),
                       objgen::op_rows(ws.rayin, RAYIN, (long)a->R * RAYIN), false);
      hipLaunchKernelGGL(feat_rowstats_kernel, dim3((a->R + 15) / 16, a->K), dim3(256), 0, st, a->params,
                         (long)a->p_stride, d.L.of_b, C, a->R, a->gt_feat, ws.rayin);
    }
    if (bf16) launch_train_bf16(d, stream, true);
    else { choose_flat(d, a->K, 4); launch_train32(d, stream, true); }
    if (hipGetLastError() != hipSuccess) return OBJNERF_ELAUNCH;
    const long nr = (long)a->K * a->R;
    int gpo = 2 * objnerf_num_cu() / a->K;
    if (gpo < 1) gpo = 1;
    if (gpo > 16) gpo = 16;
    const size_t part_room = ((size_t)((char*)ws.X2 - (char*)ws.X1) / 4 + (size_t)a->K * a->R * XCOLS) / (size_t)a->K;
    while (gpo > 1 && (size_t)gpo * ((size_t)C * XCOLS + XCOLS * XCOLS) > part_room) --gpo;
    const bool one_pass = C == 512 && (size_t)gpo * ((size_t)C * XCOLS + XCOLS * XCOLS) <= part_room;
    int Gfin = 1;
    const float *Tsrc = ws.Tm, *Msrc = ws.mom;
    if (one_pass) {
      float* Tpart = ws.X1;
      float* Mpart = ws.X1 + (size_t)a->K * gpo * C * XCOLS;
      hipLaunchKernelGGL(feat_post_kernel, dim3(gpo, a->K), dim3(512), 0, st, C, a->R, a->gt_feat, ws.rayfeat, Tpart, Mpart);
      Gfin = gpo; Tsrc = Tpart; Msrc = Mpart;
    } else {
      hipLaunchKernelGGL(feat_scale_kernel, dim3((unsigned)((nr * XCOLS + 255) / 256)), dim3(256), 0, st, nr, ws.rayfeat, ws.X1, ws.X2);
      (void)hipMemsetAsync(ws.Tm, 0, ((size_t)a->K * C * XCOLS + (size_t)a->K * XCOLS * XCOLS) * 4, st);
      objgen::wgrad_f32(stream, a->K, C, XCOLS, a->R, objgen::op_cols(a->gt_feat, C, (long)a->R * C),
                        objgen::op_rows(ws.X1, XCOLS, (long)a->R * XCOLS), objgen::op_rows(ws.Tm, XCOLS, (long)C * XCOLS),
                        ws.parts_t, objgen::wgrad_parts_floats(a->K, C, XCOLS, a->R));
      objgen::wgrad_f32(stream, a->K, XCOLS, XCOLS, a->R, objgen::op_cols(ws.X2, XCOLS, (long)a->R * XCOLS),
                        objgen::op_rows(ws.rayfeat, RAYFEAT, (long)a->R * RAYFEAT),
                        objgen::op_rows(ws.mom, XCOLS, (long)XCOLS * XCOLS), ws.parts_m,
                        objgen::wgrad_parts_floats(a->K, XCOLS, XCOLS, a->R));
    }
    if (one_pass && pre_one) {
      fin_T = Tsrc; fin_M = Msrc; fin_G = Gfin;
    } else {
      hipLaunchKernelGGL(feat_finish_kernel, dim3((C * XCOLS + 255) / 256, a->K), dim3(256), 0, st, a->params,
                         (long)a->p_stride, d.L.of_w, d.L.of_b, C, Tsrc, Msrc, a->grads, Gfin);
    }
  } else if (bf16) {
    launch_train_bf16(d, stream, false);
  } else {
    choose_flat(d, a->K, 4);
    launch_train32(d, stream, false);
  }
  if (hipGetLastError() != hipSuccess) return OBJNERF_ELAUNCH;
  const long P = offs[OBJNERF_N_TENSORS];
  dim3 fg((unsigned)((P + 256 * FIN_EPT - 1) / (256 * FIN_EPT)), (unsigned)a->K);
  FinalizeArgs fa;
  fa.slab = d.slab; fa.loss_part = d.loss_part; fa.K = a->K; fa.G = d.G; fa.P = P; fa.slab_stride = (long)ps;
  fa.p_stride = (long)a->p_stride;
  fa.ng_lo = feat ? P : d.L.fl_w; fa.ng_hi = feat ? P : d.L.pe_b;
  fa.ext_lo = feat ? d.L.of_w : P; fa.ext_hi = feat ? d.L.pe_b : P;
  fa.grads = a->grads; fa.loss_terms = a->loss_terms; fa.status = a->status;
  fa.flat_nwg = d.flat_nwg; fa.NT = d.NT; fa.Gs = d.Gs;
  fa.params = nullptr; fa.m = fa.v = nullptr; fa.flags = a->flags; fa.steps = nullptr; fa.bank = 0;
  fa.lo1 = offs[OBJNERF_T_CL_W]; fa.lo2 = offs[OBJNERF_T_FL_W]; fa.hi2 = offs[OBJNERF_T_PE_B];
  fa.lr = fa.b1 = fa.b2 = fa.wd = 0.0; fa.eps = 0.f;
  fa.counts_in = self_counts ? a->counts : nullptr; fa.flags_out = const_cast<int*>(a->flags);
  fa.Tpart = fin_T; fa.Mpart = fin_M; fa.head_w = ws.head_snap; fa.Gfin = fin_G; fa.C = C; fa.of_w = d.L.of_w; fa.of_b = d.L.of_b;
  if (a->optim) {
    const objnerf_adamw_args* o = a->optim;
    fa.params = const_cast<float*>(a->params); fa.m = o->exp_avg; fa.v = o->exp_avg_sq; fa.steps = o->group_steps;
    fa.bank = o->bank; fa.lr = (double)o->lr; fa.b1 = (double)o->beta1; fa.b2 = (double)o->beta2;
    fa.wd = (double)o->weight_decay; fa.eps = o->eps;
  }
  hipLaunchKernelGGL(finalize_kernel, fg, dim3(256), 0, st, fa);
  if (hipGetLastError() != hipSuccess) return OBJNERF_ELAUNCH;
  return OBJNERF_OK;
}

int objnerf_eval_points(const objnerf_net* net, int32_t K, int64_t N, const float* params, int64_t p_stride,
                        const float* scale, const float* pts, float* out_alpha, float* out_color, float* out_hfeat,
                        float* out_clip, void* stream) {
  (void)hipGetLastError();
  if (!net || !params || !scale || !pts || !out_alpha || !out_color || K <= 0 || N <= 0) return OBJNERF_EINVAL;
  if (net->hidden != 32 || net->n_freqs != 6) return OBJNERF_ENOTSUP;
  if (out_clip && !out_hfeat) return OBJNERF_EINVAL;
  return eval_launch(net, K, N, params, p_stride, scale, pts, nullptr, out_alpha, out_color, out_hfeat, out_clip,
                     stream);
}

size_t objnerf_eval_workspace_bytes(const objnerf_net* net, int32_t K, int64_t N) {
  if (!net || K <= 0 || N <= 0 || net->hidden == 32) return 0;
  return objgen::eval_workspace_bytes(net, K, (long)N);
}

int objnerf_eval_points_ws(const objnerf_net* net, int32_t K, int64_t N, const float* params, int64_t p_stride,
                           const float* scale, const float* pts, float* out_alpha, float* out_color, float* out_hfeat,
                           float* out_clip, void* workspace, size_t workspace_bytes, void* stream) {
  (void)hipGetLastError();
  if (!net || !params || !scale || !pts || !out_alpha || !out_color || K <= 0 || N <= 0) return OBJNERF_EINVAL;
  if (net->hidden == 32)
    return objnerf_eval_points(net, K, N, params, p_stride, scale, pts, out_alpha, out_color, out_hfeat, out_clip, stream);
  return objgen::eval_points(net, K, (long)N, params, (long)p_stride, scale, pts, out_alpha, out_color, out_hfeat,
                             out_clip, workspace, workspace_bytes, stream);
}

int objnerf_mlp_forward(const objnerf_net* net, int32_t K, int64_t N, const float* params, int64_t p_stride,
                        const float* emb, float* out_alpha, float* out_color, float* out_hfeat, float* out_clip,
                        void* stream) {
  (void)hipGetLastError();
  if (!net || !params || !emb || !out_alpha || !out_color || K <= 0 || N <= 0) return OBJNERF_EINVAL;
  if (net->hidden != 32 || net->n_freqs != 6) return OBJNERF_ENOTSUP;
  if (out_clip && !out_hfeat) return OBJNERF_EINVAL;
  return eval_launch(net, K, N, params, p_stride, nullptr, nullptr, emb, out_alpha, out_color, out_hfeat, out_clip,
                     stream);
}

int objnerf_mlp_forward_ws(const objnerf_net* net, int32_t K, int64_t N, const float* params, int64_t p_stride,
                           const float* emb, float* out_alpha, float* out_color, float* out_hfeat, float* out_clip,
                           void* workspace, size_t workspace_bytes, void* stream) {
  (void)hipGetLastError();
  if (!net || !params || !emb || !out_alpha || !out_color || K <= 0 || N <= 0) return OBJNERF_EINVAL;
  if (net->hidden == 32)
    return objnerf_mlp_forward(net, K, N, params, p_stride, emb, out_alpha, out_color, out_hfeat, out_clip, stream);
  return objgen::eval_points(net, K, (long)N, params, (long)p_stride, nullptr, nullptr, out_alpha, out_color, out_hfeat,
                             out_clip, workspace, workspace_bytes, stream, emb);
}

size_t objnerf_mlp_backward_workspace_bytes(const objnerf_net* net, int32_t K, int64_t N, int32_t with_clip) {
  if (!net || K <= 0 || N <= 0) return 0;
  return objgen::mlp_backward_workspace_bytes(net, K, (long)N, with_clip);
}

int objnerf_mlp_backward_ws(const objnerf_net* net, int32_t K, int64_t N, const float* params, int64_t p_stride,
                            const float* emb, const float* d_alpha, const float* d_color, const float* d_clip,
                            float* grads, float* d_emb, void* workspace, size_t workspace_bytes, void* stream) {
  (void)hipGetLastError();
  if (!net || !params || !emb || !d_alpha || !d_color || !grads || !d_emb || K <= 0 || N <= 0) return OBJNERF_EINVAL;
  return objgen::mlp_backward(net, K, (long)N, params, (long)p_stride, emb, d_alpha, d_color, d_clip, grads, d_emb, workspace,
                              workspace_bytes, stream);
}

int objnerf_embed_bwd(const objnerf_net* net, int32_t K, int64_t N, const float* params, int64_t p_stride,
                      const float* scale, const float* pts, const float* d_emb, float* d_B, float* scratch, void* stream) {
  (void)hipGetLastError();
  if (!net || !params || !scale || !pts || !d_emb || !d_B || !scratch || K <= 0 || N <= 0) return OBJNERF_EINVAL;
// ... 5 lines not shown
```

openobj_amd/csrc/objnerf_train32.hip:

```cpp
#include <mutex>
#include <type_traits>
#define OBJ32_PIN 1
#include "objnerf_mlp32.h"
#include "objnerf_train_common.h"
#include "../../include/objnerf_hip.h"

using namespace obj32n;
using namespace objtrain;

#if !defined(OBJ_LAZY_HEADS) && !defined(OBJ_BUTTERFLY_HEADS)
#define OBJ_LAZY_HEADS
#endif

#ifndef OBJ32_ABL
#define OBJ32_ABL 0
#endif
#define TILE_SYNC() do { if (!((OBJ32_ABL) & 2)) __syncthreads(); } while (0)
#ifndef OBJ32_WG_UNROLL_FAST
#define OBJ32_WG_UNROLL_FAST 16
#endif

#ifndef OBJ32_PHASE_LANE
#define OBJ32_PHASE_LANE 0x11
#endif
// ... 44 lines not shown
  if ((OBJ32_ABL) & 8) return;
  dT = (const float*)__builtin_assume_aligned(dT, 8);
  aT = (const float*)__builtin_assume_aligned(aT, 8);
#pragma unroll UNR
  for (int st = 0; st < 32; st += 2) {
    const f32x2 b = *reinterpret_cast<const f32x2*>(aT + st);
    const f32x2 a0 = *reinterpret_cast<const f32x2*>(dT + st);
    acc0 = OBJ_MFMA(a0[0], b[0], acc0);
    acc0 = OBJ_MFMA(a0[1], b[1], acc0);
  }
}

template <int UNR = 8>
__device__ __forceinline__ void wg_quarter(f32x4& acc0, const float* dT, const float* aT, const int st0) {
  if ((OBJ32_ABL) & 8) return;
  dT = (const float*)__builtin_assume_aligned(dT, 8);
  aT = (const float*)__builtin_assume_aligned(aT, 8);
#pragma unroll UNR
  for (int st = st0; st < st0 + 16; st += 2) {
    const f32x2 b = *reinterpret_cast<const f32x2*>(aT + st);
    const f32x2 a0 = *reinterpret_cast<const f32x2*>(dT + st);
    acc0 = OBJ_MFMA(a0[0], b[0], acc0);
    acc0 = OBJ_MFMA(a0[1], b[1], acc0);
  }
}

template <int UNR = 8>
__device__ __forceinline__ void wg_pair_ray(f32x4& acc0, f32x4& acc1, const float* dT, const float* aT, const bool odd) {
  if ((OBJ32_ABL) & 8) return;
  dT = (const float*)__builtin_assume_aligned(dT, 8);
  aT = (const float*)__builtin_assume_aligned(aT, 8);
#pragma unroll UNR
  for (int j = 0; j < 16; ++j) {
    const f32x2 b2 = *reinterpret_cast<const f32x2*>(aT + 2 * j);
    const f32x2 a02 = *reinterpret_cast<const f32x2*>(dT + 2 * j);
    const f32x2 a12 = *reinterpret_cast<const f32x2*>(dT + 16 * STG_LD + 2 * j);
    const float b = odd ? b2[1] : b2[0];
    const float a0 = odd ? a02[1] : a02[0];
    const float a1 = odd ? a12[1] : a12[0];
    acc0 = OBJ_MFMA(a0, b, acc0);
    OBJ32_PIN_MFMA();
    acc1 = OBJ_MFMA(a1, b, acc1);
    OBJ32_PIN_MFMA();
  }
}

__device__ __forceinline__ void wr_pair(float* slab, const f32x4& a0, const f32x4& a1, const int g, const int col,
                                        const int w_off, const int ncols, const int b_off) {
#pragma unroll
  for (int r = 0; r < 4; ++r) {
    const int o0 = 4 * g + r, o1 = 16 + 4 * g + r;
    if (col >= 0) {
      slab[w_off + o0 * ncols + col] = a0[r];
      slab[w_off + o1 * ncols + col] = a1[r];
    } else if (col == BIAS_COL && b_off >= 0) {
      slab[b_off + o0] = a0[r];
      slab[b_off + o1] = a1[r];
    }
  }
}

__device__ __forceinline__ void wr_half(float* slab, const f32x4& a0, const int half, const int g, const int col,
                                        const int w_off, const int ncols, const int b_off) {
#pragma unroll
  for (int r = 0; r < 4; ++r) {
    const int o = 16 * half + 4 * g + r;
    if (col >= 0) slab[w_off + o * ncols + col] = a0[r];
    else if (col == BIAS_COL && b_off >= 0) slab[b_off + o] = a0[r];
  }
}

#ifdef PHASE_TIMING
__device__ unsigned long long g_phase32[8][24];
#define PT_INIT() unsigned long long pt_acc[18]; for (int i_ = 0; i_ < 18; ++i_) pt_acc[i_] = 0; \
  unsigned long long pt_t0 = __builtin_amdgcn_s_memtime()
#define PT(i) do { const unsigned long long t_ = __builtin_amdgcn_s_memtime(); pt_acc[i] += t_ - pt_t0; pt_t0 = t_; } while (0)
#define PT_FLUSH() do { if (blockIdx.x == 0 && lane == 0) for (int i_ = 0; i_ < 18; ++i_) g_phase32[w][i_] = pt_acc[i_]; } while (0)
#else
#define PT_INIT() do {} while (0)
#define PT(i) do {} while (0)
#define PT_FLUSH() do {} while (0)
#endif

template <bool FEAT>
struct Lay {
  static constexpr int IMG = img_floats(FEAT);
  static constexpr int ROWS = FEAT ? 160 : STG_ROWS;
  static constexpr int LDS_FLOATS = IMG + SM_FLOATS + ROWS * STG_LD;
  static constexpr int A_H3 = FEAT ? 0 : 96, A_DHC = FEAT ? 80 : 128, A_DHF = 112, A_DH4 = FEAT ? 80 : 160;
  static constexpr int C_DH2 = FEAT ? 128 : 160;
  static_assert(LDS_FLOATS * 4 <= 163840, "LDS budget");
  static_assert((IMG * 4) % 16 == 0, "staging area alignment");
};
constexpr int F_SW = 144 * STG_LD;
constexpr int F_GFH = F_SW + TS;
constexpr int F_GOF = F_GFH + 16 * 32;
static_assert(F_GOF + 32 <= 160 * STG_LD && OFF_FHB + 64 * NWAVE <= 80 * STG_LD, "feature aliases");

template <bool FEAT, bool MASKS, int SS>
__global__ __launch_bounds__(NTHR) void train_fused32_kernel(const TrainDev a) {
  typedef Lay<FEAT> LY;
  constexpr int IMG = LY::IMG;
  constexpr bool FAST = !FEAT;
  constexpr int WGU = (!FEAT && !MASKS && SS == 64) ? OBJ32_WG_UNROLL_FAST : 8;
  constexpr bool SKIP = !FEAT && !MASKS;
  constexpr bool RAYS = SKIP && SS == 64;
  constexpr bool DEAD_ZEROS = !RAYS;
  extern __shared__ __attribute__((aligned(16))) float lds[];
  const int tid = threadIdx.x;
  int lane = tid & 63;
  const int w = __builtin_amdgcn_readfirstlane(tid >> 6);
  int c = lane & 15, g = lane >> 4;
  float* sv = lds + sv_base(FEAT);
  float* s_alpha = lds + IMG;
  float* s_col = s_alpha + TS;
  float* stg = lds + IMG + SM_FLOATS;

  const long T_flat = (long)a.K * a.NT;
  long cur = a.flat_nwg ? T_flat * blockIdx.x / a.flat_nwg : 0;
  const long cur_end = a.flat_nwg ? T_flat * (blockIdx.x + 1) / a.flat_nwg : 1;
  bool first_seg = true;
  while (cur < cur_end) {
  int k, t0, t1, tstep, sslot;
  if (a.flat_nwg) {
    k = (int)(cur / a.NT);
    t0 = (int)(cur - (long)k * a.NT);
    const long rem = cur_end - cur;
    t1 = (long)t0 + rem < (long)a.NT ? (int)(t0 + rem) : a.NT;
    tstep = 1;
    sslot = (int)blockIdx.x - flat_wg_of(T_flat, a.flat_nwg, (long)k * a.NT);
    cur += t1 - t0;
  } else {
    k = blockIdx.x / a.G; t0 = blockIdx.x % a.G; t1 = a.NT; tstep = a.G; sslot = t0;
    cur = cur_end;
  }
  const int n_slots = a.flat_nwg ? a.Gs : a.G;
  if (!first_seg) __syncthreads();
  first_seg = false;

  stage_weights32(lds, a.params + (long)k * a.p_stride, a.L, FEAT, tid, NTHR);
  for (int i = tid; i < LY::ROWS * STG_LD; i += NTHR) stg[i] = 0.0f;
  __syncthreads();

  const float scale = a.scale[k];
  const int S = SS ? SS : a.S, R = a.R, TR = SS ? TS / SS : a.TR;
  const float n1 = (float)a.counts[2 * k], n2 = (float)a.counts[2 * k + 1];
  int bflag0, bflag1;
  batch_flags(a, bflag0, bflag1);
  float inv1 = bflag0 ? 0.0f : 1.0f / (n1 + 1e-10f);
  float inv2 = bflag1 ? 0.0f : 1.0f / (n2 + 1e-10f);
  if (SKIP) {
    inv1 = __builtin_bit_cast(float, __builtin_amdgcn_readfirstlane(__builtin_bit_cast(int, inv1)));
    inv2 = __builtin_bit_cast(float, __builtin_amdgcn_readfirstlane(__builtin_bit_cast(int, inv2)));
  }

  const float* wf = (const float*)__builtin_assume_aligned(lds + 4 * g * WROW + out_pos(c), 8);
  const float* wt0 = (const float*)__builtin_assume_aligned(lds + c * WROW + 8 * g + 4 * (g & 1), 16);
  const float* wt1 = (const float*)__builtin_assume_aligned(lds + c * WROW + 8 * g + 4 * (1 - (g & 1)), 16);
  float* stg_lane = stg + (4 * g) * STG_LD + 16 * w + c;
  const float* lane_rd = stg + c * STG_LD + 32 * g;
  int slot = 16 * w + c;
  auto phase_lane = [&](const int site) {
    if (!SKIP || !(((OBJ32_PHASE_LANE) >> site) & 1)) return;
    asm volatile("v_mbcnt_lo_u32_b32 %0, -1, 0\n\tv_mbcnt_hi_u32_b32 %0, -1, %0" : "=v"(lane));
    c = lane & 15; g = lane >> 4;
    slot = 16 * w + c;
    wf = (const float*)__builtin_assume_aligned(lds + 4 * g * WROW + out_pos(c), 8);
    wt0 = (const float*)__builtin_assume_aligned(lds + c * WROW + 8 * g + 4 * (g & 1), 16);
    wt1 = (const float*)__builtin_assume_aligned(lds + c * WROW + 8 * g + 4 * (1 - (g & 1)), 16);
    stg_lane = stg + (4 * g) * STG_LD + 16 * w + c;
    lane_rd = stg + c * STG_LD + 32 * g;
  };

  f32x4 accA0 = zero4(), accA1 = zero4(), accB0 = zero4(), accB1 = zero4(), accC0 = zero4(), accC1 = zero4();
  f32x4 accA2 = zero4(), accC2 = zero4();
#ifdef OBJ_LAZY_HEADS
  constexpr bool LAZY_H = !FEAT;
#else
  constexpr bool LAZY_H = false;
#endif
  float hW[4][8];
#pragma unroll
  for (int s_ = 0; s_ < 8; ++s_) hW[0][s_] = hW[1][s_] = hW[2][s_] = hW[3][s_] = 0.f;
  float gS0 = 0.f;
  float gS1 = 0.f;
#ifdef OBJ_LAZY_BIAS
  float bS[2][8];
#pragma unroll
  for (int s_ = 0; s_ < 8; ++s_) bS[0][s_] = bS[1][s_] = 0.f;
#else
  float gS2 = 0.f;
#endif
  float g_hb = 0.f;
  float dB[6][3];
#pragma unroll
  for (int i = 0; i < 6; ++i) dB[i][0] = dB[i][1] = dB[i][2] = 0.f;
  float l_d = 0.f, l_c = 0.f, l_o = 0.f, l_f = 0.f;

  auto fetch_point = [&](const int tile_, const int slot_, float& x, float& y, float& z_) {
    const int q_ = slot_ / S, si_ = slot_ - q_ * S;
    const int ray_ = tile_ * TR + q_;
    x = 0.f; y = 0.f; z_ = 0.f;
    if (tile_ < t1 && q_ < TR && ray_ < a.R) {
      const long rr = (long)k * a.R + ray_;
      if (a.pts) {
        const float* p = a.pts + (rr * S + si_) * 3;
        x = p[0]; y = p[1]; z_ = p[2];
      } else {
        const float zz = a.z[rr * S + si_];
        const float* o = a.origins + rr * 3;
        const float* d = a.dirs + rr * 3;
        x = (o[0] + d[0] * zz) - a.obj_center;
        y = (o[1] + d[1] * zz) - a.obj_center;
        z_ = (o[2] + d[2] * zz) - a.obj_center;
      }
    }
  };
  const bool rows_mode = SS ? true : seg_is_rows(S);
  const SegRows seg_rows = SegRows::make(rows_mode ? S : 64, lane);
// ... 580 lines not shown
    d_h2 = zero32();
    mma_t32<FAST>(d_h2, wt0, wt1, R_CAT, d_h3);
    d_h2 = relu_mask32(d_h2, act.h2);
#ifdef OBJ_LAZY_BIAS
#pragma unroll
    for (int tt = 0; tt < 2; ++tt)
#pragma unroll
      for (int r = 0; r < 4; ++r) bS[0][4 * tt + r] += d_h2.t[tt][r];
#else
    float pa2_[8];
#pragma unroll
    for (int tt = 0; tt < 2; ++tt)
#pragma unroll
      for (int r = 0; r < 4; ++r) pa2_[4 * tt + r] = d_h2.t[tt][r];
    {
      const float sv8 = slot_sums8(pa2_, c);
      gS2 += (c < 8) ? sv8 : 0.0f;
      asm volatile("" : "+v"(gS2));
    }
#endif
    d_h1 = zero32();
    mma_t32<FAST>(d_h1, wt0, wt1, R_M1, d_h2);
    d_h1 = relu_mask32(d_h1, act.h1);
#pragma unroll
    for (int T = 0; T < 6; ++T) {
      f32x4 d_x = zero4();
      mma_t16<FAST>(d_x, wt0, wt1, R_CAT + 32 + 16 * T, d_h3);
      mma_t16<FAST>(d_x, wt0, wt1, R_IN + 16 * T, d_h1);
      st_T16(stg_lane, 32 + 16 * T, pe32_x1_tile_fb(pe, T, g, d_x, dps[T]));
    }
#pragma unroll
    for (int i = 0; i < 6; ++i) {
      dB[i][0] = fmaf(dps[i], pe.t[0], dB[i][0]);
      dB[i][1] = fmaf(dps[i], pe.t[1], dB[i][1]);
      dB[i][2] = fmaf(dps[i], pe.t[2], dB[i][2]);
    }
    }
    PT(10);
    PT(11);
    TILE_SYNC();
    PT(12);
    phase_lane(5);
    if (RAYS) wg_round(accB0, accB1, rays_live(false), 128, 16 * w);
    else if (!tile_dead()) wg_pair<WGU>(accB0, accB1, lane_rd + 128 * STG_LD, lane_rd + (16 * w) * STG_LD);
    PT(13);
    TILE_SYNC();
    phase_lane(6);
    fetch_point(tile + tstep, slot, nx, ny, nz);
    fetch_labels(tile + tstep, nlb0, nlb1);
    if (wave_dead()) {
      if (DEAD_ZEROS) {
        st_zero<2>(stg_lane, 0);
        st_zero<4>(stg_lane, 128);
      }
    } else {
    st_T32(stg_lane, 0, act.h1);
    st_T32(stg_lane, 128, d_h1);
    if (!FEAT) st_T32(stg_lane, LY::C_DH2, d_h2);
    }
    PT(14);
    TILE_SYNC();
    PT(15);
    phase_lane(7);
    if (FEAT) {
      if (w < 6) wg_pair<WGU>(accC0, accC1, lane_rd + 128 * STG_LD, lane_rd + (32 + 16 * w) * STG_LD);
      TILE_SYNC();
      st_T32(stg_lane, LY::C_DH2, d_h2);
      TILE_SYNC();
      wg_quarter<WGU>(accC2, lane_rd + (LY::C_DH2 + 16 * ((w >> 1) & 1)) * STG_LD, lane_rd + (16 * (w >> 2)) * STG_LD,
                 16 * (w & 1));
      TILE_SYNC();
    } else if (RAYS) {
      wg_round(accC0, accC1, rays_live(false), (w < 6) ? 128 : 160, (w < 6) ? 32 + 16 * w : 16 * (w - 6));
    } else if (!tile_dead()) {
      const int dTr = (w < 6) ? 128 : 160;
      const int aTr = (w < 6) ? 32 + 16 * w : 16 * (w - 6);
      wg_pair<WGU>(accC0, accC1, lane_rd + dTr * STG_LD, lane_rd + aTr * STG_LD);
    }
    PT(16);
    PT(17);
  }
  PT_FLUSH();

  float* slab = a.slab + ((long)k * n_slots + sslot) * a.slab_stride;
  const Layout& L = a.L;
  {
    int t_, g_;
    auto cl_col = [&](const int rho) {
      int col = rho;
      if (rho >= H) { kappa_tg(rho - H, t_, g_); col = x2_col(t_, g_); if (col >= 0) col += H; }
      return col;
    };
    if (FEAT) {
      if (w < 5) wr_pair(slab, accA0, accA1, g, cl_col(16 * w + c), L.cl_w, H + OBJ_E2, L.cl_b);
      else wr_pair(slab, accA0, accA1, g, cl_col(16 * (w - 5) + c), L.fl_w, H + OBJ_E2, L.fl_b);
      const int half = w & 1, t2 = (w & 3) >> 1;
      if (w < 4) wr_half(slab, accA2, half, g, cl_col(48 + 16 * t2 + c), L.fl_w, H + OBJ_E2, L.fl_b);
      else wr_half(slab, accA2, half, g, 16 * t2 + c, L.m2_w, H, -1);
    } else if (w < 5) {
      wr_pair(slab, accA0, accA1, g, cl_col(16 * w + c), L.cl_w, H + OBJ_E2, L.cl_b);
    } else if (w < 7) {
      wr_pair(slab, accA0, accA1, g, 16 * (w - 5) + c, L.m2_w, H, -1);
    }
    {
      const int rho = 16 * w + c;
      int col = rho;
      if (rho >= H) { kappa_tg(rho - H, t_, g_); col = x1_col(t_, g_); if (col >= 0) col += H; }
      wr_pair(slab, accB0, accB1, g, col, L.cat_w, H + OBJ_E1, L.cat_b);
    }
    if (w < 6) {
      kappa_tg(16 * w + c, t_, g_);
      wr_pair(slab, accC0, accC1, g, x1_col(t_, g_), L.in_w, OBJ_E1, L.in_b);
    } else if (!FEAT) {
      wr_pair(slab, accC0, accC1, g, 16 * (w - 6) + c, L.m1_w, H, -1);
    }
  }
  if (FEAT) {
    __syncthreads();
    float* xch = stg + (w >> 1) * 256 + 4 * lane;
    if (w & 1) *reinterpret_cast<f32x4*>(xch) = accC2;
    __syncthreads();
    if (!(w & 1)) {
      accC2 += *reinterpret_cast<const f32x4*>(xch);
      wr_half(slab, accC2, (w >> 1) & 1, g, 16 * (w >> 2) + c, L.m1_w, H, -1);
    }
  }
  __syncthreads();
  float* red = stg;
  constexpr int NRED32 = 6 * 32 + 4 + 4 + 72;
  {
    float* mine = red + w * NRED32;
    {
      const int s = c & 7;
      const int row = 16 * (s >> 2) + 4 * g + (s & 3);
      if (LAZY_H) {
#pragma unroll
        for (int s_ = 0; s_ < 8; ++s_) {
          const int rw = 16 * (s_ >> 2) + 4 * g + (s_ & 3);
          const float v2 = dpp_rowsum16(hW[0][s_]), v3 = dpp_rowsum16(hW[1][s_]);
          const float v4 = dpp_rowsum16(hW[2][s_]), v5 = dpp_rowsum16(hW[3][s_]);
          if (c == 0) { mine[64 + rw] = v2; mine[96 + rw] = v3; mine[128 + rw] = v4; mine[160 + rw] = v5; }
        }
      } else {
        if (c < 8) { mine[64 + row] = gS0; mine[128 + row] = gS1; }
        else { mine[96 + row] = gS0; mine[160 + row] = gS1; }
      }
#ifdef OBJ_LAZY_BIAS
#pragma unroll
      for (int s_ = 0; s_ < 8; ++s_) {
        const int rw = 16 * (s_ >> 2) + 4 * g + (s_ & 3);
        const float v0 = dpp_rowsum16(bS[0][s_]), v1 = dpp_rowsum16(bS[1][s_]);
        if (c == 0) { mine[rw] = v0; mine[32 + rw] = v1; }
      }
#else
      mine[(c < 8 ? 0 : 32) + row] = gS2;
#endif
    }
    const float hb = dpp_rowsum16(g_hb);
    if (c == 0) mine[192 + g] = hb;
    const float e0 = wave_sum64(l_d), e1 = wave_sum64(l_c), e2 = wave_sum64(l_o);
    const float e3 = FEAT ? wave_sum64(l_f) : 0.0f;
    if (lane == 0) { mine[196] = e0; mine[197] = e1; mine[198] = e2; mine[199] = e3; }
#pragma unroll
    for (int i = 0; i < 6; ++i)
#pragma unroll
      for (int x = 0; x < 3; ++x) {
        const float v = dpp_rowsum16(dB[i][x]);
        if (c == 0) mine[200 + 12 * i + 3 * g + x] = v;
      }
  }
  __syncthreads();
  for (int i = tid; i < NRED32; i += NTHR) {
    float v = 0.f;
#pragma unroll
    for (int ww = 0; ww < NWAVE; ++ww) v += red[ww * NRED32 + i];
    if (i < 32) slab[L.m1_b + i] = v;
    else if (i < 64) slab[L.m2_b + i - 32] = v;
    else if (i < 96) slab[L.a_w + i - 64] = v;
    else if (i < 192) slab[L.oc_w + i - 96] = v;
    else if (i == 192) slab[L.a_b] = v;
    else if (i < 196) slab[L.oc_b + i - 193] = v;
    else if (i < 200) a.loss_part[((long)k * n_slots + sslot) * 4 + (i - 196)] = v;
    else if (i - 200 < 3 * OBJ_NDIR) slab[L.pe_b + (i - 200)] = v;
  }
  }
}

}

namespace objtrain {

size_t fused32_lds_bytes() { return (size_t)Lay<false>::LDS_FLOATS * 4; }

void launch_train32(const TrainDev& d, void* stream, bool feat) {
  constexpr int n0 = Lay<false>::LDS_FLOATS * 4, n1 = Lay<true>::LDS_FLOATS * 4;
  objnerf_once_per_device([] {
    (void)hipFuncSetAttribute((const void*)train_fused32_kernel<false, false, 64>, hipFuncAttributeMaxDynamicSharedMemorySize, n0);
    (void)hipFuncSetAttribute((const void*)train_fused32_kernel<false, false, 0>, hipFuncAttributeMaxDynamicSharedMemorySize, n0);
    (void)hipFuncSetAttribute((const void*)train_fused32_kernel<false, true, 0>, hipFuncAttributeMaxDynamicSharedMemorySize, n0);
    (void)hipFuncSetAttribute((const void*)train_fused32_kernel<true, false, 0>, hipFuncAttributeMaxDynamicSharedMemorySize, n1);
    (void)hipFuncSetAttribute((const void*)train_fused32_kernel<true, false, 64>, hipFuncAttributeMaxDynamicSharedMemorySize, n1);
    (void)hipFuncSetAttribute((const void*)train_fused32_kernel<true, true, 0>, hipFuncAttributeMaxDynamicSharedMemorySize, n1);
  });
  const dim3 grid(d.flat_nwg ? d.flat_nwg : d.K * d.G), blk(NTHR);
  hipStream_t st = (hipStream_t)stream;
  if (feat) {
    if (d.relu_masks || d.emb_debug) hipLaunchKernelGGL((train_fused32_kernel<true, true, 0>), grid, blk, n1, st, d);
    else if (d.S == 64) hipLaunchKernelGGL((train_fused32_kernel<true, false, 64>), grid, blk, n1, st, d);
    else hipLaunchKernelGGL((train_fused32_kernel<true, false, 0>), grid, blk, n1, st, d);
  } else if (d.relu_masks || d.emb_debug) hipLaunchKernelGGL((train_fused32_kernel<false, true, 0>), grid, blk, n0, st, d);
  else if (d.S == 64) hipLaunchKernelGGL((train_fused32_kernel<false, false, 64>), grid, blk, n0, st, d);
  else hipLaunchKernelGGL((train_fused32_kernel<false, false, 0>), grid, blk, n0, st, d);
}

}

#ifdef PHASE_TIMING
extern "C" int objnerf_debug_phase32(unsigned long long* out_host) {
  if (hipDeviceSynchronize() != hipSuccess) return -1;
  return hipMemcpyFromSymbol(out_host, HIP_SYMBOL(g_phase32), sizeof(unsigned long long) * 8 * 24) == hipSuccess ? 0 : -1;
}
#endif
```

openobj_amd/csrc/objnerf_train_common.h:

```cpp
#pragma once
#include "objnerf_mlp.h"

namespace objtrain {
using namespace obj32;

constexpr int TS = 128;
constexpr int NWAVE = 8;
constexpr int NTHR = 64 * NWAVE;
constexpr int STG_LD = 130;
constexpr int STG_ROWS = 192;
constexpr int SM_FLOATS = 4 * TS;
constexpr int NRED = 6 * 32 + 4 + 4;

struct TrainDev {
  int K, R, S, G, TR, NT;
  float color_scaling, opacity_scaling, feat_scaling, obj_center;
  const float* params; long p_stride; const float* scale;
  const float* pts; const float* origins; const float* dirs; const float* z;
  const float* gt_depth; const float* gt_rgb; const uint8_t* labels; const float* gt_feat;
  const int* counts; const int* flags;
  int derive_flags;
  float* slab;
  long slab_stride;
  float* loss_part;
  int flat_nwg, Gs;
  const float* rayin;
  const float* gram;
  float* rayfeat;
  uint8_t* relu_masks;
  float* emb_debug;
  Layout L;
};
constexpr int RAYIN = 34, GRAM = 1088, RAYFEAT = 36;
__device__ __forceinline__ void batch_flags(const TrainDev& a, int& f0, int& f1) {
  if (!a.derive_flags) { f0 = a.flags[0]; f1 = a.flags[1]; return; }
  int e0 = 0, e1 = 0;
  for (int k = threadIdx.x & 63; k < a.K; k += 64) { e0 |= a.counts[2 * k] == 0; e1 |= a.counts[2 * k + 1] == 0; }
  f0 = __ballot(e0) != 0; f1 = __ballot(e1) != 0;
}
__host__ __device__ inline int flat_wg_of(const long T, const int nwg, const long x) { return (int)(((x + 1) * nwg - 1) / T); }
constexpr int HF_LD = 33;
constexpr int OFF_GBUF = TS * HF_LD;
constexpr int OFF_FHB = OFF_GBUF + 32 * 33 + 64;
static_assert(OFF_FHB + 64 * NWAVE <= 80 * STG_LD, "feat lds aliases");


__device__ __forceinline__ void write_relu_mask(uint8_t* dst , const int layer,
                                                const int g, const T32& act, const bool valid) {
  unsigned n0 = 0, n1 = 0;
#pragma unroll
  for (int r = 0; r < 4; ++r) {
    n0 |= (act.t[0][r] > 0.0f ? 1u : 0u) << r;
    n1 |= (act.t[1][r] > 0.0f ? 1u : 0u) << r;
  }
  const unsigned v = (n0 << (4 * (g & 1))) | (n1 << (8 + 4 * (g & 1)));
  const unsigned o = v | (unsigned)__shfl_xor((int)v, 16, 64);
  if (valid && (g & 1) == 0) {
    dst[layer * 4 + (g >> 1)] = (uint8_t)(o & 0xff);
    dst[layer * 4 + 2 + (g >> 1)] = (uint8_t)(o >> 8);
  }
}

size_t fused32_lds_bytes();
void launch_train32(const TrainDev& d, void* stream, bool feat);

size_t bf16_lds_bytes();
void launch_train_bf16(const TrainDev& d, void* stream, bool feat);
size_t bf16v2_lds_bytes();
void launch_train_bf16_v2(const TrainDev& d, void* stream);
void launch_train_bf16_v2f(const TrainDev& d, void* stream);

}
```

openobj_amd/ops.py:

```python
from __future__ import annotations

import ctypes as C
import os
from dataclasses import dataclass
from typing import Dict, List, Optional, Sequence, Tuple

import numpy as np
import torch

from . import _lib
from ._lib import AdamWArgs, LossArgs, Net, ObjnerfError, SampleArgs, TRAIN_SELF_COUNTS, TrainArgs, check, lib

EMB1, EMB2, N_DIRS = 87, 42, 21
TENSOR_NAMES = [
    "in_layer.0.weight", "in_layer.0.bias", "mid1.0.0.weight", "mid1.0.0.bias",
    "cat_layer.0.weight", "cat_layer.0.bias", "mid2.0.0.weight", "mid2.0.0.bias",
    "out_alpha.weight", "out_alpha.bias", "color_linear.0.weight", "color_linear.0.bias",
    "out_color.weight", "out_color.bias", "clip_linear.0.weight", "clip_linear.0.bias",
    "out_clip.weight", "out_clip.bias", "B_layer.weight",
]
FEAT_TENSORS = (14, 15, 16, 17)


def tensor_shapes(hidden: int, feat_dim: int = 512) -> List[Tuple[int, ...]]:
    H, Cc = hidden, feat_dim
    return [(H, EMB1), (H,), (H, H), (H,), (H, H + EMB1), (H,), (H, H), (H,), (1, H), (1,),
            (H, EMB2 + H), (H,), (3, H), (3,), (H, EMB2 + H), (H,), (Cc, H), (Cc,), (N_DIRS, 3)]


def _ptr(t: Optional[torch.Tensor]) -> Optional[int]:
    if t is None:
        return None
    return t.data_ptr()


def _stream() -> int:
    return torch.cuda.current_stream().cuda_stream


def _req(t: torch.Tensor, dtype, name: str) -> torch.Tensor:
    if not t.is_cuda:
        raise _lib.ObjnerfError(f"{name}: expected a GPU tensor (there is no CPU path)")
    if t.dtype != dtype:
        raise _lib.ObjnerfError(f"{name}: expected {dtype}, got {t.dtype}")
    if not t.is_contiguous():
        t = t.contiguous()
    return t


@dataclass
class NetShape:
    hidden: int = 32
    feat_dim: int = 512
    n_freqs: int = 6

    def c(self) -> Net:
        return Net(self.hidden, self.feat_dim, self.n_freqs, 0)


class ParamArena:

    def __init__(self, K: int, net: NetShape, device):
        self.K, self.net = K, net
        self.offsets, self.p_stride = _lib.param_layout(net.hidden, net.feat_dim, net.n_freqs)
        self.P = self.offsets[-1]
        self.shapes = tensor_shapes(net.hidden, net.feat_dim)
        self.params = torch.zeros(K, self.p_stride, dtype=torch.float32, device=device)
        self.scale = torch.full((K,), 2.0, dtype=torch.float32, device=device)
        self.version = 0

    def set_scale(self, value: float) -> None:
        key = (float(value), self.scale._version)
        if getattr(self, "_scale_set", None) == key:
            return
        self.scale.fill_(float(value))
        self._scale_set = (float(value), self.scale._version)

    def state_version(self):
        return (self.version, self.params._version, self.scale._version)

    def owns(self, t: torch.Tensor) -> bool:
        lo = self.params.data_ptr()
        return t.device == self.params.device and lo <= t.data_ptr() < lo + self.params.numel() * 4

    def views(self, buf: Optional[torch.Tensor] = None) -> List[torch.Tensor]:
        buf = self.params if buf is None else buf
        out = []
        for i, shp in enumerate(self.shapes):
            n = 1
            for s in shp:
                n *= s
            out.append(buf[:, self.offsets[i]:self.offsets[i] + n].view(self.K, *shp))
        return out

# ... 265 lines not shown

LAYERWISE_WORKSPACE_BUDGET = int(float(os.environ.get("OBJNERF_WORKSPACE_BUDGET_GIB", "64")) * (1 << 30))


def precision_bits(p) -> int:
    if p in (False, None, "fp32"):
        return 0
    if p in (True, "bf16"):
        return 1
    if p == "fp16":
        return 4
    raise ValueError("precision must be fp32 / bf16 / fp16, not {!r}".format(p))


class StreamContext:

    def __init__(self, device):
        self.device = torch.device(device)
        h = C.c_void_p()
        with torch.cuda.device(self.device):
            check(lib().objnerf_context_create(C.byref(h)), "objnerf_context_create")
        self.handle = h

    def __del__(self):
        h, self.handle = getattr(self, "handle", None), None
        if h:
            try:
                torch.cuda.synchronize(self.device)
                lib().objnerf_context_destroy(h)
            except Exception:
                pass


class TrainWorkspace:

    def __init__(self, arena: ParamArena, K: int, R: int, S: int, with_feat: bool, layerwise: bool = False,
                 budget: Optional[int] = None, precision=None, context: Optional["StreamContext"] = None):
        layerwise = layerwise or precision_bits(precision) == 4
        dev = arena.params.device
        net = arena.net.c()
        wf = int(with_feat) | (2 if layerwise else 0) | (4 if precision_bits(precision) in (1, 4) else 0)
        budget = LAYERWISE_WORKSPACE_BUDGET if budget is None else budget
        self.k_chunk = K
        nbytes = lib().objnerf_train_workspace_bytes(C.byref(net), K, R, S, wf)
        if (arena.net.hidden != 32 or S > 64 or layerwise) and nbytes > budget and K > 1:
            per_obj = lib().objnerf_train_workspace_bytes(C.byref(net), 1, R, S, wf)
            self.k_chunk = max(1, min(K, int(budget // max(1, per_obj))))
            nbytes = lib().objnerf_train_workspace_bytes(C.byref(net), self.k_chunk, R, S, wf)
        if nbytes == 0:
            raise _lib.ObjnerfError("objnerf_train_workspace_bytes returned 0")
        self.nbytes = int(nbytes)
        uses_context = (arena.net.hidden != 32 or S > 64 or layerwise) and dev.type == "cuda"
        self.context = (context if context is not None else StreamContext(dev)) if uses_context else None
        self.buf = torch.empty(self.nbytes, dtype=torch.uint8, device=dev)
        self.lanes = 1
        self.buf2 = None
        if (self.k_chunk < K and dev.type == "cuda" and arena.net.hidden == 256 and precision_bits(precision) in (1, 4)
                and not (layerwise and precision_bits(precision) != 4) and S in (32, 64, 128)
                and os.environ.get("OBJNERF_ONE_LANE", "0") != "1"):
            free, total = torch.cuda.mem_get_info(dev)
            if free - self.nbytes > max(total // 4, 16 << 30):
                self.buf2 = torch.empty(self.nbytes, dtype=torch.uint8, device=dev)
                with torch.cuda.device(dev):
                    self.sides = [torch.cuda.Stream(device=dev), torch.cuda.Stream(device=dev)]
                    self.ev_in, self.ev_out = torch.cuda.Event(), [torch.cuda.Event(), torch.cuda.Event()]
                self.lanes = 2
        self.grads = torch.zeros_like(arena.params)
        self.loss_terms = torch.zeros(K, 4, device=dev)
        self.status = torch.zeros(1, dtype=torch.int32, device=dev)
        self.status_chunks = torch.zeros((K + self.k_chunk - 1) // self.k_chunk, dtype=torch.int32, device=dev)
        self.counts = torch.zeros(K, 2, dtype=torch.int32, device=dev)
        self.flags = torch.zeros(2, dtype=torch.int32, device=dev)
        self.key = self.make_key(K, R, S, with_feat, precision)

    @staticmethod
    def make_key(K, R, S, with_feat, precision=None):
        return (K, R, S, bool(with_feat), precision_bits(precision))


def train_step(arena: ParamArena, ws: TrainWorkspace, batch: Dict[str, torch.Tensor], color_scaling=5.0,
               opacity_scaling=10.0, feat_scaling=5.0, with_feat=False, obj_center=0.0,
               global_flags: Optional[torch.Tensor] = None, global_counts: Optional[torch.Tensor] = None,
               bf16: bool = False, layerwise: bool = False, relu_masks: Optional[torch.Tensor] = None,
               emb_debug: Optional[torch.Tensor] = None, optim=None) -> None:
    z = _req(batch["z"], torch.float32, "z")
    K, R, S = z.shape
    labels = _req(batch["labels"], torch.uint8, "labels")
    pts = batch.get("pts")
    pts = _req(pts, torch.float32, "pts") if pts is not None else None
    origins = _req(batch["origins"], torch.float32, "origins") if pts is None else None
    dirs = _req(batch["dirs"], torch.float32, "dirs") if pts is None else None
    gt_depth = _req(batch["gt_depth"], torch.float32, "gt_depth")
    gt_rgb = _req(batch["gt_rgb"], torch.float32, "gt_rgb")
    gt_feat = _req(batch["gt_feat"], torch.float32, "gt_feat") if with_feat else None
    st = _stream()
    self_counts = global_flags is None and global_counts is None
    if not self_counts and (global_flags is None or global_counts is None):
        check(lib().objnerf_label_counts(K, R, _ptr(labels), _ptr(ws.counts), _ptr(ws.flags), st),
              "objnerf_label_counts")
    flags = ws.flags
    if global_flags is not None:
        flags = _req(global_flags, torch.int32, "global_flags")
    counts = ws.counts
    if global_counts is not None:
        counts = _req(global_counts, torch.int32, "global_counts")
    net = arena.net.c()
    mode = precision_bits(bf16) | (2 if layerwise else 0)
    if relu_masks is not None:
        relu_masks = _req(relu_masks, torch.uint8, "relu_masks")
        if tuple(relu_masks.shape) != (K, R, S, 6, arena.net.hidden // 8):
            raise ObjnerfError("relu_masks must be uint8 [K,R,S,6,hidden/8]")
    if emb_debug is not None:
        emb_debug = _req(emb_debug, torch.float32, "emb_debug")
        if tuple(emb_debug.shape) != (K, R, S, EMB1 + EMB2):
            raise ObjnerfError("emb_debug must be float32 [K,R,S,129]")
    kc = getattr(ws, "k_chunk", K)
    ctx = ws.context.handle if getattr(ws, "context", None) is not None else None
    if kc >= K:
        oa = None
        if optim is not None:
            if optim.arena is not arena:
                raise ObjnerfError("train_step: optim must be the optimiser of `arena`")
            oa = AdamWArgs(_ptr(optim.exp_avg), _ptr(optim.exp_avg_sq), _ptr(optim._banks), int(optim._bank), 0,
                           optim.lr, optim.betas[0], optim.betas[1], optim.eps, optim.weight_decay, 0.0)
        a = TrainArgs(K, R, S, mode | (TRAIN_SELF_COUNTS if self_counts else 0), color_scaling, opacity_scaling,
                      feat_scaling, obj_center, _ptr(arena.params),
                      arena.p_stride, _ptr(arena.scale), _ptr(pts), _ptr(origins), _ptr(dirs), _ptr(z), _ptr(gt_depth),
                      _ptr(gt_rgb), _ptr(labels), _ptr(gt_feat), _ptr(counts), _ptr(flags), _ptr(ws.grads),
                      _ptr(ws.loss_terms), _ptr(ws.status), _ptr(ws.buf), ws.nbytes, _ptr(relu_masks), ctx, _ptr(emb_debug),
                      C.addressof(oa) if oa is not None else None)
        check(lib().objnerf_train_step(C.byref(net), C.byref(a), st), "objnerf_train_step")
        if optim is not None:
            optim._bank ^= 1
            arena.version += 1
        return
    if self_counts:
        check(lib().objnerf_label_counts(K, R, _ptr(labels), _ptr(ws.counts), _ptr(ws.flags), st),
              "objnerf_label_counts")
    sl = lambda t, k0, k1: None if t is None else t[k0:k1]
    two = getattr(ws, "lanes", 1) == 2 and relu_masks is None and emb_debug is None
    if two:
        main = torch.cuda.current_stream(z.device)
        ws.ev_in.record(main)
        for sd in ws.sides:
            sd.wait_event(ws.ev_in)
    for ci, k0 in enumerate(range(0, K, kc)):
        k1 = min(K, k0 + kc)
        buf = ws.buf2 if (two and (ci & 1)) else ws.buf
        sth = ws.sides[ci & 1].cuda_stream if two else st
        a = TrainArgs(k1 - k0, R, S, mode, color_scaling, opacity_scaling, feat_scaling, obj_center,
                      _ptr(arena.params[k0:k1]), arena.p_stride, _ptr(arena.scale[k0:k1]), _ptr(sl(pts, k0, k1)),
                      _ptr(sl(origins, k0, k1)), _ptr(sl(dirs, k0, k1)), _ptr(z[k0:k1]), _ptr(gt_depth[k0:k1]),
                      _ptr(gt_rgb[k0:k1]), _ptr(labels[k0:k1]), _ptr(sl(gt_feat, k0, k1)), _ptr(counts[k0:k1]),
                      _ptr(flags), _ptr(ws.grads[k0:k1]), _ptr(ws.loss_terms[k0:k1]), _ptr(ws.status_chunks[ci:ci + 1]),
                      _ptr(buf), ws.nbytes, _ptr(sl(relu_masks, k0, k1)), ctx, _ptr(sl(emb_debug, k0, k1)), None)
        check(lib().objnerf_train_step(C.byref(net), C.byref(a), sth), "objnerf_train_step")
    if two:
        for sd, ev in zip(ws.sides, ws.ev_out):
            ev.record(sd)
            main.wait_event(ev)
    merge_status(ws.status_chunks, out=ws.status)
    if optim is not None:
        optim.step(ws.grads, arena.has_grad_mask(with_feat), flags=flags)


def adamw_step(arena: ParamArena, grads: torch.Tensor, exp_avg: torch.Tensor, exp_avg_sq: torch.Tensor,
               has_grad: Optional[torch.Tensor], step: int, lr: float, weight_decay: float, beta1=0.9, beta2=0.999,
               eps=1e-8, params: Optional[torch.Tensor] = None) -> None:
    p = arena.params if params is None else params
    if params is None:
        arena.version += 1
    check(lib().objnerf_adamw_step(arena.K, arena.P, arena.p_stride, _ptr(p), _ptr(grads), _ptr(exp_avg),
                                   _ptr(exp_avg_sq), _ptr(has_grad), step, lr, beta1, beta2, eps, weight_decay,
                                   _stream()), "objnerf_adamw_step")


def adamw_step_flags(arena: ParamArena, grads: torch.Tensor, exp_avg: torch.Tensor, exp_avg_sq: torch.Tensor,
                     has_grad: Optional[torch.Tensor], flags: torch.Tensor, group_steps: torch.Tensor, bank: int,
                     lr: float, weight_decay: float, beta1=0.9, beta2=0.999, eps=1e-8,
                     params: Optional[torch.Tensor] = None) -> None:
    p = arena.params if params is None else params
    if params is None:
        arena.version += 1
    flags = _req(flags, torch.int32, "flags")
    group_steps = _req(group_steps, torch.int32, "group_steps")
    if group_steps.numel() != 6 or bank not in (0, 1):
        raise ObjnerfError("adamw_step_flags: group_steps must be int32[2, 3], bank 0 or 1")
    o = arena.offsets
    check(lib().objnerf_adamw_step_flags(arena.K, arena.P, arena.p_stride, _ptr(p), _ptr(grads), _ptr(exp_avg),
                                         _ptr(exp_avg_sq), _ptr(has_grad), _ptr(flags), _ptr(group_steps), int(bank),
                                         int(o[10]), int(o[14]), int(o[18]), lr, beta1, beta2, eps, weight_decay, _stream()),
          "objnerf_adamw_step_flags")


def ingest_frame(rgb, depth, inst, t_wc, items) -> None:
    import numpy as np
    from ._lib import IngestItem
    rgb = _req(rgb, torch.uint8, "rgb")
    depth = _req(depth, torch.float32, "depth")
    inst = _req(inst, torch.int32, "inst")
    t_wc = _req(t_wc, torch.float32, "t_wc")
    W, H = depth.shape
    arr = (IngestItem * len(items))()
    for i, ((rgbs_b, depth_b, twc_b, bbox_b), slot, obj_id, box) in enumerate(items):
        if rgbs_b.shape[1:] != (W, H, 4) or depth_b.shape[1:] != (W, H) or not 0 <= slot < rgbs_b.shape[0]:
            raise ObjnerfError("ingest_frame: store / frame shapes do not match")
        arr[i] = IngestItem(rgbs_b.data_ptr(), depth_b.data_ptr(), twc_b.data_ptr(), bbox_b.data_ptr(), int(slot),
                            int(obj_id), (C.c_float * 4)(*[float(v) for v in box]))
    host = torch.from_numpy(np.frombuffer(arr, dtype=np.uint8).copy())
    dev_items = host.to(rgb.device)
    check(lib().objnerf_ingest_frame(W, H, _ptr(rgb), _ptr(depth), _ptr(inst), _ptr(t_wc), len(items), _ptr(dev_items),
                                     _stream()), "objnerf_ingest_frame")


def ingest_frame_crops(rgb, depth, inst, t_wc, items, outside) -> None:
    import numpy as np
    from ._lib import IngestCropItem, KfCrops
    from .kf_store import crop_rect
    rgb = _req(rgb, torch.uint8, "rgb")
    depth = _req(depth, torch.float32, "depth")
    inst = _req(inst, torch.int32, "inst")
    t_wc = _req(t_wc, torch.float32, "t_wc")
    outside = _req(outside, torch.int32, "outside")
    W, H = depth.shape
    if outside.numel() < len(items):
        raise ObjnerfError("ingest_frame_crops: one `outside` counter per item expected")
    if len({(id(st), int(slot)) for st, slot, _, _ in items}) != len(items):
        raise ObjnerfError("ingest_frame_crops: a slot is written twice")
    for st, slot, _, box in items:
        if (st.W, st.H) != (W, H) or not 0 <= slot < st.F or len(box) != 4:
            raise ObjnerfError("ingest_frame_crops: store / frame shapes do not match")
    rects = [crop_rect(box, W, H) for _, _, _, box in items]
    for (st, slot, _, _), rect in zip(items, rects):
        st.reserve(int(slot), rect)
    arr = (IngestCropItem * len(items))()
    for i, (st, slot, obj_id, box) in enumerate(items):
        _req(st.arena, torch.uint8, "arena"); _req(st.rect, torch.int32, "rect")
        _req(st.t_wc, torch.float32, "t_wc_batch"); _req(st.bbox, torch.float32, "bbox")
        if rects[i][2] * rects[i][3] > st.cap or st.arena.numel() != st.F * st.cap * 8:
            raise ObjnerfError("ingest_frame_crops: the crop does not fit its store")
        arr[i] = IngestCropItem(KfCrops(*st.descriptor()), int(slot), int(obj_id),
                                (C.c_float * 4)(*[float(v) for v in box]), (C.c_int32 * 4)(*rects[i]))
    dev_items = torch.from_numpy(np.frombuffer(arr, dtype=np.uint8).copy()).to(rgb.device)
    check(lib().objnerf_ingest_frame_crops(W, H, _ptr(rgb), _ptr(depth), _ptr(inst), _ptr(t_wc), len(items),
                                           _ptr(dev_items), _ptr(outside), _stream()), "objnerf_ingest_frame_crops")


def keyframe_table(stores) -> torch.Tensor:
# ... 1670 lines not shown
```

Before: 24.12 million rays/s.

## Balance flat tile partition across workgroups using label-dependent cost model

Replaces the uniform split of flattened (object, tile) work across workgroups with cost-weighted bounds computed from per-ray label pairs. A new label-count kernel also runs a prefix sum over estimated tile costs and writes workgroup boundaries, and the train kernel and finalize reduction read these bounds with one slab slot per segment. The goal is to even out workgroup runtimes when objects have skewed label distributions, in exchange for a heavier counting kernel and a binary search in finalize. It applies by default only for the fp32, no-feature, S=64 self-counts path.

```diff
diff --git a/include/objnerf_hip.h b/include/objnerf_hip.h
--- a/include/objnerf_hip.h
+++ b/include/objnerf_hip.h
@@ -152,6 +152,7 @@
 #define OBJNERF_TRAIN_FP16 4
 #define OBJNERF_TRAIN_LAYERWISE 2
 #define OBJNERF_TRAIN_SELF_COUNTS 8
+#define OBJNERF_TRAIN_COUNT_PARTITION 16
 struct objnerf_context;
 int objnerf_context_create(struct objnerf_context** out);
 int objnerf_context_destroy(struct objnerf_context* ctx);
@@ -179,6 +180,8 @@
 size_t objnerf_train_workspace_bytes(const objnerf_net* net, int32_t K, int32_t R, int32_t S,
                                      int32_t with_feat);
 int objnerf_train_step(const objnerf_net* net, const objnerf_train_args* a, void* stream);
+int64_t objnerf_train_flat_bounds(const objnerf_net* net, int32_t K, int32_t R, int32_t S, int32_t mode, int32_t with_feat,
+                                  int32_t* nwg_out);
 
 int objnerf_adamw_step(int32_t K, int64_t P, int64_t p_stride, float* params, const float* grads,
                        float* exp_avg, float* exp_avg_sq, const uint8_t* has_grad, int32_t step,
diff --git a/openobj_amd/_lib.py b/openobj_amd/_lib.py
--- a/openobj_amd/_lib.py
+++ b/openobj_amd/_lib.py
@@ -63,6 +63,7 @@
 
 TRAIN_BF16 = 1
 TRAIN_SELF_COUNTS = 8
+TRAIN_COUNT_PARTITION = 16
 
 
 class AdamWArgs(C.Structure):
@@ -234,6 +235,8 @@
     "objnerf_train_workspace_bytes": (C.c_size_t, [C.POINTER(Net), C.c_int32, C.c_int32, C.c_int32,
                                                    C.c_int32]),
     "objnerf_train_step": (C.c_int, [C.POINTER(Net), C.POINTER(TrainArgs), C.c_void_p]),
+    "objnerf_train_flat_bounds": (C.c_int64, [C.POINTER(Net), C.c_int32, C.c_int32, C.c_int32, C.c_int32, C.c_int32,
+                                              C.POINTER(C.c_int32)]),
     "objnerf_adamw_step": (C.c_int, [C.c_int32, C.c_int64, C.c_int64, C.c_void_p, C.c_void_p, C.c_void_p,
                                      C.c_void_p, C.c_void_p, C.c_int32, C.c_float, C.c_float, C.c_float,
                                      C.c_float, C.c_float, C.c_void_p]),
diff --git a/openobj_amd/csrc/objnerf_generic.h b/openobj_amd/csrc/objnerf_generic.h
--- a/openobj_amd/csrc/objnerf_generic.h
+++ b/openobj_amd/csrc/objnerf_generic.h
@@ -12,6 +12,8 @@
                       int64_t colour_lo, int64_t feature_lo, int64_t feature_hi, int64_t ng_lo, int64_t ng_hi, float lr,
                       float beta1, float beta2, float eps, float weight_decay, void* stream);
 int label_counts_only(int32_t K, int32_t R, const uint8_t* labels, int32_t* counts, void* stream);
+int label_counts_bounds(int32_t K, int32_t R, const uint8_t* labels, int32_t* counts, int32_t* bounds, int32_t nwg,
+                        void* stream);
 }
 
 namespace objgen {
diff --git a/openobj_amd/csrc/objnerf_misc.hip b/openobj_amd/csrc/objnerf_misc.hip
--- a/openobj_amd/csrc/objnerf_misc.hip
+++ b/openobj_amd/csrc/objnerf_misc.hip
@@ -4,6 +4,7 @@
 #include "objnerf_generic.h"
 #include "objnerf_step_tail.h"
 #include "objnerf_boxray.h"
+#include "objnerf_train_common.h"
 
 namespace {
 
@@ -122,6 +123,123 @@
     } else {
       if (a == 0) atomicOr(&flags[0], 1);
       if (b == 0) atomicOr(&flags[1], 1);
+    }
+  }
+}
+
+__device__ __forceinline__ void load_labels16(const uint8_t* p, const int n, unsigned (&wd)[4]) {
+  if (n >= 16 && ((uintptr_t)p & 15) == 0) {
+    const uint4 v = *reinterpret_cast<const uint4*>(p);
+    wd[0] = v.x; wd[1] = v.y; wd[2] = v.z; wd[3] = v.w;
+  } else {
+#pragma unroll
+    for (int i = 0; i < 4; ++i) {
+      unsigned x = 0;
+#pragma unroll
+      for (int j = 0; j < 4; ++j) x |= (unsigned)(4 * i + j < n ? p[4 * i + j] : (uint8_t)2) << (8 * j);
+      wd[i] = x;
+    }
+  }
+}
+__device__ __forceinline__ unsigned pair_index2(const unsigned wd) { return wd * 3u + (wd >> 8); }
+constexpr int LB_WG = 512;
+__global__ __launch_bounds__(LB_WG) void label_bounds_kernel(int K, int R, const uint8_t* labels, int* counts, int* bounds,
+                                                             int nwg) {
+  __shared__ int lb_lut[16], lb_fold[LB_WG / 64], lb_c[2 * (LB_WG / 64)];
+  __shared__ long long lb_w[2 * (LB_WG / 64)];
+  const int k = blockIdx.x, tid = threadIdx.x, lane = tid & 63, w = tid >> 6;
+  const int NT = (R + 1) >> 1, nch = (R + 15) >> 4;
+  const int c22 = objtrain::flat_tile_cost(2, 2);
+  if (tid < 16) lb_lut[tid] = tid < 9 ? objtrain::flat_tile_cost(tid / 3, tid % 3) : c22;
+  __syncthreads();
+  auto chunk_cost = [&](const unsigned (&wd)[4]) {
+    int s = 0;
+#pragma unroll
+    for (int i = 0; i < 4; ++i) {
+      const unsigned x = pair_index2(wd[i]);
+      s += lb_lut[x & 15u] + lb_lut[(x >> 16) & 15u];
+    }
+    return s;
+  };
+  long long sW = 0, sP = 0;
+  const int n_items = K * nch, mine_from = k * nch;
+  if ((R & 15) == 0 && ((uintptr_t)labels & 15) == 0) {
+    const uint4* lv = reinterpret_cast<const uint4*>(labels);
+#pragma unroll 8
+    for (int i = tid; i < n_items; i += LB_WG) {
+      const uint4 v = lv[i];
+      const unsigned wd[4] = {v.x, v.y, v.z, v.w};
+      const int s = chunk_cost(wd);
+      sW += s;
+      sP += i < mine_from ? s : 0;
+    }
+  } else {
+    for (int i = tid; i < n_items; i += LB_WG) {
+      const int j = i / nch, c = i - j * nch;
+      unsigned wd[4];
+      load_labels16(labels + (long)j * R + 16 * c, R - 16 * c, wd);
+      const int s = chunk_cost(wd);
+      sW += s;
+      sP += i < mine_from ? s : 0;
+    }
+  }
+#pragma unroll
+  for (int d = 32; d >= 1; d >>= 1) { sW += __shfl_xor(sW, d, 64); sP += __shfl_xor(sP, d, 64); }
+  if (lane == 0) { lb_w[2 * w] = sW; lb_w[2 * w + 1] = sP; }
+  const uint8_t* lk = labels + (long)k * R;
+  const int cpt = (nch + LB_WG - 1) / LB_WG;
+  const int ch0 = tid * cpt, ch1 = ch0 + cpt < nch ? ch0 + cpt : nch;
+  int mine = 0, c1 = 0, c2 = 0;
+  for (int c = ch0; c < ch1; ++c) {
+    unsigned wd[4];
+    load_labels16(lk + 16 * c, R - 16 * c, wd);
+    mine += chunk_cost(wd);
+    const int tiles = NT - 8 * c < 8 ? NT - 8 * c : 8;
+    mine -= (8 - tiles) * c22;
+    const int n = R - 16 * c < 16 ? R - 16 * c : 16;
+#pragma unroll
+    for (int i = 0; i < 16; ++i) {
+      const int l = (wd[i >> 2] >> (8 * (i & 3))) & 0xff;
+      c1 += (i < n) & (l == 1);
+      c2 += (i < n) & (l != 2);
+    }
+  }
+  int total;
+  const int before = wg_exclusive<LB_WG>(mine, lb_fold, total);
+#pragma unroll
+  for (int d = 32; d >= 1; d >>= 1) { c1 += __shfl_xor(c1, d, 64); c2 += __shfl_xor(c2, d, 64); }
+  if (lane == 0) { lb_c[2 * w] = c1; lb_c[2 * w + 1] = c2; }
+  long long W = 0, P = 0;
+#pragma unroll
+  for (int q = 0; q < LB_WG / 64; ++q) { W += lb_w[2 * q]; P += lb_w[2 * q + 1]; }
+  const long long pad = (long long)(8 * nch - NT) * c22;
+  W -= pad * K;
+  P -= pad * k;
+  __syncthreads();
+  if (tid < 2) {
+    int t = 0;
+    for (int q = 0; q < LB_WG / 64; ++q) t += lb_c[2 * q + tid];
+    counts[2 * k + tid] = t;
+  }
+  if (k == K - 1 && tid == 0) bounds[nwg] = K * NT;
+  if (ch0 >= ch1) return;
+  long long E = P + before;
+  long long b = (E * nwg + W - 1) / W;
+  long long tgt = b < nwg ? W * b / nwg : W;
+  for (int c = ch0; c < ch1; ++c) {
+    unsigned wd[4];
+    load_labels16(lk + 16 * c, R - 16 * c, wd);
+#pragma unroll
+    for (int i = 0; i < 8; ++i) {
+      const int t = 8 * c + i;
+      if (t >= NT) break;
+      const unsigned x = pair_index2(wd[i >> 1]);
+      E += lb_lut[(x >> (16 * (i & 1))) & 15u];
+      while (b < nwg && tgt < E) {
+        bounds[b] = k * NT + t;
+        ++b;
+        tgt = W * b / nwg;
+      }
     }
   }
 }
@@ -782,6 +900,14 @@
   CHECK_LAUNCH();
   return OBJNERF_OK;
 }
+int label_counts_bounds(int32_t K, int32_t R, const uint8_t* labels, int32_t* counts, int32_t* bounds, int32_t nwg,
+                        void* stream) {
+  CLEAR_STALE();
+  if (K <= 0 || R <= 0 || !labels || !counts || !bounds || nwg <= 0 || (long)K * R >= (1L << 31)) return OBJNERF_EINVAL;
+  hipLaunchKernelGGL(label_bounds_kernel, dim3(K), dim3(LB_WG), 0, (hipStream_t)stream, K, R, labels, counts, bounds, nwg);
+  CHECK_LAUNCH();
+  return OBJNERF_OK;
+}
 int adamw_flags_range(int32_t K, int64_t P, int64_t p_stride, float* params, const float* grads, float* exp_avg,
                       float* exp_avg_sq, const uint8_t* has_grad, const int32_t* flags, int32_t* group_steps, int32_t bank,
                       int64_t colour_lo, int64_t feature_lo, int64_t feature_hi, int64_t ng_lo, int64_t ng_hi, float lr,
diff --git a/openobj_amd/csrc/objnerf_train.hip b/openobj_amd/csrc/objnerf_train.hip
--- a/openobj_amd/csrc/objnerf_train.hip
+++ b/openobj_amd/csrc/objnerf_train.hip
@@ -24,6 +24,7 @@
   long ng_lo, ng_hi, ext_lo, ext_hi;
   float* grads; float* loss_terms; int* status;
   int flat_nwg, NT, Gs;
+  const int* bounds;
   float* params; float* m; float* v; const int* flags; int* steps; int bank;
   long lo1, lo2, hi2;
   double lr, b1, b2, wd; float eps;
@@ -61,13 +62,29 @@
       for (int g = 0; g < a.Gfin; ++g) v += a.Mpart[((long)k * a.Gfin + g) * XCOLS * XCOLS + e];
       s_M[e] = v;
     }
-  if (a.params || first || head_blk) __syncthreads();
-  int G = a.G;
-  if (a.flat_nwg) {
+  __shared__ int s_tab[FLAT_BOUNDS_MAX_NWG + 1];
+  if (a.bounds)
+    for (int i = threadIdx.x; i <= a.flat_nwg; i += 256) s_tab[i] = a.bounds[i];
+  if (a.params || first || head_blk || a.bounds) __syncthreads();
+  auto flat_range = [&](const int kk, int& b0, int& b1) {
+    const long lo = (long)kk * a.NT, hi = lo + a.NT;
+    int l = 0, r = a.flat_nwg - 1;
+    while (l < r) { const int m = (l + r) >> 1; if (s_tab[m + 1] > lo) r = m; else l = m + 1; }
+    b0 = l;
+    l = 0; r = a.flat_nwg - 1;
+    while (l < r) { const int m = (l + r + 1) >> 1; if (s_tab[m] < hi) l = m; else r = m - 1; }
+    b1 = l;
+  };
+  int G = a.G, g0 = 0;
+  if (a.bounds) {
+    int b1;
+    flat_range(k, g0, b1);
+    G = b1 + 1;
+  } else if (a.flat_nwg) {
     const long T = (long)a.K * a.NT;
     G = flat_wg_of(T, a.flat_nwg, (long)(k + 1) * a.NT - 1) - flat_wg_of(T, a.flat_nwg, (long)k * a.NT) + 1;
   }
-  const int stride = a.flat_nwg ? a.Gs : a.G;
+  const int stride = a.bounds ? 1 : a.flat_nwg ? a.Gs : a.G;
   float s[FIN_EPT];
   bool live[FIN_EPT], slabbed[FIN_EPT];
 #pragma unroll
@@ -78,6 +95,16 @@
     s[e] = 0.f;
   }
   const float* sl0 = a.slab + (long)k * stride * a.slab_stride + i0;
+  if (a.bounds) {
+    for (int g = g0; g < G; ++g) {
+      const bool has = s_tab[g] < s_tab[g + 1];
+      float t[FIN_EPT];
+#pragma unroll
+      for (int e = 0; e < FIN_EPT; ++e) t[e] = slabbed[e] ? sl0[(long)g * a.slab_stride + 256 * e] : 0.f;
+#pragma unroll
+      for (int e = 0; e < FIN_EPT; ++e) s[e] = has ? s[e] + t[e] : s[e];
+    }
+  } else
   for (int g = 0; g < G; ++g) {
     float t[FIN_EPT];
 #pragma unroll
@@ -133,13 +160,20 @@
     int bad = 0;
     for (int e = threadIdx.x; e < 4 * a.K; e += blockDim.x) {
       const int kk = e >> 2;
-      int Gk = a.G;
-      if (a.flat_nwg) {
+      int Gk = a.G, gk0 = 0;
+      if (a.bounds) {
+        int b1;
+        flat_range(kk, gk0, b1);
+        Gk = b1 + 1;
+      } else if (a.flat_nwg) {
         const long T = (long)a.K * a.NT;
         Gk = flat_wg_of(T, a.flat_nwg, (long)(kk + 1) * a.NT - 1) - flat_wg_of(T, a.flat_nwg, (long)kk * a.NT) + 1;
       }
       float sl = 0.f;
-      for (int g = 0; g < Gk; ++g) sl += a.loss_part[((long)kk * stride + g) * 4 + (e & 3)];
+      for (int g = gk0; g < Gk; ++g) {
+        if (a.bounds && s_tab[g] >= s_tab[g + 1]) continue;
+        sl += a.loss_part[((long)kk * stride + g) * 4 + (e & 3)];
+      }
       a.loss_terms[e] = sl;
       bad |= loss_status_bits(sl);
     }
@@ -578,6 +612,15 @@
   const long gs = ((long)d.NT * cu + T - 1) / T + 1;
   if (cost_flat < cost_strided && gs <= grid_cap(K)) { d.flat_nwg = cu; d.Gs = (int)gs; }
 }
+static bool flat_count_forced() {
+  static const bool v = [] { const char* e = getenv("OBJNERF_FLAT_COUNT"); return e && e[0] == '1'; }();
+  return v;
+}
+static bool flat_balanced(const TrainDev& d, int K, int S, int mode, bool feat, bool bf16, int64_t ps) {
+  return d.flat_nwg > 0 && !feat && !bf16 && S == 64 && (mode & OBJNERF_TRAIN_SELF_COUNTS) &&
+         !(mode & OBJNERF_TRAIN_COUNT_PARTITION) && !flat_count_forced() && d.flat_nwg <= FLAT_BOUNDS_MAX_NWG &&
+         (long)d.flat_nwg + K <= (long)K * grid_cap(K) && d.flat_nwg + 1 <= ps && (long)K * d.NT < (1L << 30);
+}
 
 struct Workspace32 {
   float* slab;
@@ -587,6 +630,7 @@
   float *Tm, *mom;
   float *parts_t, *parts_m;
   float* head_snap;
+  int32_t* flat_bounds;
   size_t bytes;
 };
 static Workspace32 workspace32(uintptr_t base, int K, int R, int C, int64_t ps, bool feat) {
@@ -606,6 +650,7 @@
     w.parts_m = take(objgen::wgrad_parts_floats(K, XCOLS, XCOLS, R));
     w.head_snap = take((size_t)K * C * XCOLS);
   }
+  w.flat_bounds = (int32_t*)(w.slab + ((size_t)K * grid_cap(K) - 1) * ps);
   return w;
 }
 
@@ -615,6 +660,24 @@
   int64_t offs[OBJNERF_N_TENSORS + 1];
   const int64_t ps = objnerf_param_layout(net, offs);
   return workspace32(0, K, R, net->feat_dim, ps, (with_feat & 1) != 0).bytes;
+}
+
+int64_t objnerf_train_flat_bounds(const objnerf_net* net, int32_t K, int32_t R, int32_t S, int32_t mode, int32_t with_feat,
+                                  int32_t* nwg_out) {
+  if (!net || K <= 0 || R <= 0 || S <= 0 || !nwg_out) return OBJNERF_EINVAL;
+  *nwg_out = 0;
+  if (net->hidden != 32 || S > 64 || (mode & (OBJNERF_TRAIN_LAYERWISE | OBJNERF_TRAIN_FP16))) return -1;
+  const bool feat = (with_feat & 1) != 0, bf16 = (mode & OBJNERF_TRAIN_BF16) != 0;
+  TrainDev d = {};
+  d.TR = TS / S;
+  d.NT = (R + d.TR - 1) / d.TR;
+  d.G = train_grid(K, d.NT);
+  if (!bf16) choose_flat(d, K, 4);
+  *nwg_out = d.flat_nwg;
+  int64_t offs[OBJNERF_N_TENSORS + 1];
+  const int64_t ps = objnerf_param_layout(net, offs);
+  if (!flat_balanced(d, K, S, mode, feat, bf16, ps)) return -1;
+  return (int64_t)(uintptr_t)workspace32(0, K, R, net->feat_dim, ps, feat).flat_bounds;
 }
 
 int objnerf_train_step(const objnerf_net* net, const objnerf_train_args* a, void* stream) {
@@ -664,10 +727,6 @@
   const bool self_counts = (a->mode & OBJNERF_TRAIN_SELF_COUNTS) != 0;
   const bool feat = a->gt_feat != nullptr;
   const bool counts_in_pre = self_counts && feat && net->feat_dim <= FEAT_PRE_MAXC && net->feat_dim % 16 == 0;
-  if (self_counts && !counts_in_pre) {
-    const int rc = objmisc::label_counts_only(a->K, a->R, a->labels, const_cast<int32_t*>(a->counts), stream);
-    if (rc) return rc;
-  }
   if (feat && (TS / a->S) > 16) return OBJNERF_ENOTSUP;
   const bool bf16 = (a->mode & OBJNERF_TRAIN_BF16) != 0;
   if (bf16 && (a->relu_masks || a->emb_debug)) return OBJNERF_ENOTSUP;
@@ -683,7 +742,16 @@
   d.TR = TS / a->S;
   d.NT = (a->R + d.TR - 1) / d.TR;
   d.G = train_grid(a->K, d.NT);
-  d.flat_nwg = 0; d.Gs = 0;
+  d.flat_nwg = 0; d.Gs = 0; d.flat_bounds = nullptr;
+  if (!bf16) choose_flat(d, a->K, 4);
+  const bool balanced = flat_balanced(d, a->K, a->S, a->mode, feat, bf16, ps);
+  if (self_counts && !counts_in_pre) {
+    const int rc = balanced ? objmisc::label_counts_bounds(a->K, a->R, a->labels, const_cast<int32_t*>(a->counts), ws.flat_bounds,
+                                                           d.flat_nwg, stream)
+                            : objmisc::label_counts_only(a->K, a->R, a->labels, const_cast<int32_t*>(a->counts), stream);
+    if (rc) return rc;
+  }
+  if (balanced) d.flat_bounds = ws.flat_bounds;
   d.color_scaling = a->color_scaling; d.opacity_scaling = a->opacity_scaling; d.feat_scaling = a->feat_scaling;
   d.obj_center = a->obj_center;
   d.params = a->params; d.p_stride = a->p_stride; d.scale = a->scale;
@@ -724,7 +792,7 @@
                          (long)a->p_stride, d.L.of_b, C, a->R, a->gt_feat, ws.rayin);
     }
     if (bf16) launch_train_bf16(d, stream, true);
-    else { choose_flat(d, a->K, 4); launch_train32(d, stream, true); }
+    else launch_train32(d, stream, true);
     if (hipGetLastError() != hipSuccess) return OBJNERF_ELAUNCH;
     const long nr = (long)a->K * a->R;
     int gpo = 2 * objnerf_num_cu() / a->K;
@@ -760,7 +828,6 @@
   } else if (bf16) {
     launch_train_bf16(d, stream, false);
   } else {
-    choose_flat(d, a->K, 4);
     launch_train32(d, stream, false);
   }
   if (hipGetLastError() != hipSuccess) return OBJNERF_ELAUNCH;
@@ -772,7 +839,7 @@
   fa.ng_lo = feat ? P : d.L.fl_w; fa.ng_hi = feat ? P : d.L.pe_b;
   fa.ext_lo = feat ? d.L.of_w : P; fa.ext_hi = feat ? d.L.pe_b : P;
   fa.grads = a->grads; fa.loss_terms = a->loss_terms; fa.status = a->status;
-  fa.flat_nwg = d.flat_nwg; fa.NT = d.NT; fa.Gs = d.Gs;
+  fa.flat_nwg = d.flat_nwg; fa.NT = d.NT; fa.Gs = d.Gs; fa.bounds = d.flat_bounds;
   fa.params = nullptr; fa.m = fa.v = nullptr; fa.flags = a->flags; fa.steps = nullptr; fa.bank = 0;
   fa.lo1 = offs[OBJNERF_T_CL_W]; fa.lo2 = offs[OBJNERF_T_FL_W]; fa.hi2 = offs[OBJNERF_T_PE_B];
   fa.lr = fa.b1 = fa.b2 = fa.wd = 0.0; fa.eps = 0.f;
diff --git a/openobj_amd/csrc/objnerf_train32.hip b/openobj_amd/csrc/objnerf_train32.hip
--- a/openobj_amd/csrc/objnerf_train32.hip
+++ b/openobj_amd/csrc/objnerf_train32.hip
@@ -150,6 +150,14 @@
 #define PT_FLUSH() do {} while (0)
 #endif
 
+#ifdef FLAT_TIMING
+constexpr int WGT_MAX = 1024;
+__device__ unsigned long long g_wgtime32[WGT_MAX][2];
+#define WGT(i) do { if (threadIdx.x == 0 && blockIdx.x < WGT_MAX) g_wgtime32[blockIdx.x][i] = wall_clock64(); } while (0)
+#else
+#define WGT(i) do {} while (0)
+#endif
+
 template <bool FEAT>
 struct Lay {
   static constexpr int IMG = img_floats(FEAT);
@@ -183,26 +191,29 @@
   float* s_alpha = lds + IMG;
   float* s_col = s_alpha + TS;
   float* stg = lds + IMG + SM_FLOATS;
+  WGT(0);
 
   const long T_flat = (long)a.K * a.NT;
-  long cur = a.flat_nwg ? T_flat * blockIdx.x / a.flat_nwg : 0;
-  const long cur_end = a.flat_nwg ? T_flat * (blockIdx.x + 1) / a.flat_nwg : 1;
+  const bool balanced = !FEAT && a.flat_bounds != nullptr;
+  long cur = !a.flat_nwg ? 0 : balanced ? (long)a.flat_bounds[blockIdx.x] : T_flat * blockIdx.x / a.flat_nwg;
+  const long cur_end = !a.flat_nwg ? 1 : balanced ? (long)a.flat_bounds[blockIdx.x + 1] : T_flat * (blockIdx.x + 1) / a.flat_nwg;
   bool first_seg = true;
   while (cur < cur_end) {
-  int k, t0, t1, tstep, sslot;
+  int k, t0, t1, tstep;
+  long seg_slot;
   if (a.flat_nwg) {
     k = (int)(cur / a.NT);
     t0 = (int)(cur - (long)k * a.NT);
     const long rem = cur_end - cur;
     t1 = (long)t0 + rem < (long)a.NT ? (int)(t0 + rem) : a.NT;
     tstep = 1;
-    sslot = (int)blockIdx.x - flat_wg_of(T_flat, a.flat_nwg, (long)k * a.NT);
+    seg_slot = balanced ? (long)blockIdx.x + k
+                        : (long)k * a.Gs + ((int)blockIdx.x - flat_wg_of(T_flat, a.flat_nwg, (long)k * a.NT));
     cur += t1 - t0;
   } else {
-    k = blockIdx.x / a.G; t0 = blockIdx.x % a.G; t1 = a.NT; tstep = a.G; sslot = t0;
+    k = blockIdx.x / a.G; t0 = blockIdx.x % a.G; t1 = a.NT; tstep = a.G; seg_slot = (long)k * a.G + t0;
     cur = cur_end;
   }
-  const int n_slots = a.flat_nwg ? a.Gs : a.G;
   if (!first_seg) __syncthreads();
   first_seg = false;
 
@@ -949,7 +960,7 @@
   }
   PT_FLUSH();
 
-  float* slab = a.slab + ((long)k * n_slots + sslot) * a.slab_stride;
+  float* slab = a.slab + seg_slot * a.slab_stride;
   const Layout& L = a.L;
   {
     int t_, g_;
@@ -1047,10 +1058,11 @@
     else if (i < 192) slab[L.oc_w + i - 96] = v;
     else if (i == 192) slab[L.a_b] = v;
     else if (i < 196) slab[L.oc_b + i - 193] = v;
-    else if (i < 200) a.loss_part[((long)k * n_slots + sslot) * 4 + (i - 196)] = v;
+    else if (i < 200) a.loss_part[seg_slot * 4 + (i - 196)] = v;
     else if (i - 200 < 3 * OBJ_NDIR) slab[L.pe_b + (i - 200)] = v;
   }
   }
+  WGT(1);
 }
 
 }
@@ -1082,6 +1094,12 @@
 
 }
 
+#ifdef FLAT_TIMING
+extern "C" int objnerf_debug_wgtime32(unsigned long long* out_host, int n) {
+  if (n < 0 || n > WGT_MAX || hipDeviceSynchronize() != hipSuccess) return -1;
+  return hipMemcpyFromSymbol(out_host, HIP_SYMBOL(g_wgtime32), sizeof(unsigned long long) * 2 * n) == hipSuccess ? 0 : -1;
+}
+#endif
 #ifdef PHASE_TIMING
 extern "C" int objnerf_debug_phase32(unsigned long long* out_host) {
   if (hipDeviceSynchronize() != hipSuccess) return -1;
diff --git a/openobj_amd/csrc/objnerf_train_common.h b/openobj_amd/csrc/objnerf_train_common.h
--- a/openobj_amd/csrc/objnerf_train_common.h
+++ b/openobj_amd/csrc/objnerf_train_common.h
@@ -24,6 +24,7 @@
   long slab_stride;
   float* loss_part;
   int flat_nwg, Gs;
+  const int* flat_bounds;
   const float* rayin;
   const float* gram;
   float* rayfeat;
@@ -39,6 +40,14 @@
   f0 = __ballot(e0) != 0; f1 = __ballot(e1) != 0;
 }
 __host__ __device__ inline int flat_wg_of(const long T, const int nwg, const long x) { return (int)(((x + 1) * nwg - 1) / T); }
+constexpr int FLAT_COST_MAX = 128;
+__host__ __device__ inline int flat_tile_cost(const int l0, const int l1) {
+  const int c0 = l1 == 0 ? 102 : l1 == 1 ? 118 : 68;
+  const int c1 = l1 == 0 ? 116 : l1 == 1 ? 128 : 84;
+  const int c2 = l1 == 0 ? 69 : l1 == 1 ? 85 : 10;
+  return l0 == 0 ? c0 : l0 == 1 ? c1 : c2;
+}
+constexpr int FLAT_BOUNDS_MAX_NWG = 1024;
 constexpr int HF_LD = 33;
 constexpr int OFF_GBUF = TS * HF_LD;
 constexpr int OFF_FHB = OFF_GBUF + 32 * 33 + 64;
diff --git a/openobj_amd/ops.py b/openobj_amd/ops.py
--- a/openobj_amd/ops.py
+++ b/openobj_amd/ops.py
@@ -9,7 +9,8 @@
 import torch
 
 from . import _lib
-from ._lib import AdamWArgs, LossArgs, Net, ObjnerfError, SampleArgs, TRAIN_SELF_COUNTS, TrainArgs, check, lib
+from ._lib import (AdamWArgs, LossArgs, Net, ObjnerfError, SampleArgs, TRAIN_COUNT_PARTITION, TRAIN_SELF_COUNTS, TrainArgs,
+                   check, lib)
 
 EMB1, EMB2, N_DIRS = 87, 42, 21
 TENSOR_NAMES = [
@@ -441,7 +442,7 @@
                opacity_scaling=10.0, feat_scaling=5.0, with_feat=False, obj_center=0.0,
                global_flags: Optional[torch.Tensor] = None, global_counts: Optional[torch.Tensor] = None,
                bf16: bool = False, layerwise: bool = False, relu_masks: Optional[torch.Tensor] = None,
-               emb_debug: Optional[torch.Tensor] = None, optim=None) -> None:
+               emb_debug: Optional[torch.Tensor] = None, optim=None, count_partition: bool = False) -> None:
     z = _req(batch["z"], torch.float32, "z")
     K, R, S = z.shape
     labels = _req(batch["labels"], torch.uint8, "labels")
@@ -464,7 +465,7 @@
     if global_counts is not None:
         counts = _req(global_counts, torch.int32, "global_counts")
     net = arena.net.c()
-    mode = precision_bits(bf16) | (2 if layerwise else 0)
+    mode = precision_bits(bf16) | (2 if layerwise else 0) | (TRAIN_COUNT_PARTITION if count_partition else 0)
     if relu_masks is not None:
         relu_masks = _req(relu_masks, torch.uint8, "relu_masks")
         if tuple(relu_masks.shape) != (K, R, S, 6, arena.net.hidden // 8):
@@ -523,6 +524,17 @@
         optim.step(ws.grads, arena.has_grad_mask(with_feat), flags=flags)
 
 
+def flat_bounds(arena: ParamArena, ws: TrainWorkspace, K: int, R: int, S: int, with_feat: bool = False,
+                count_partition: bool = False):
+    net = arena.net.c()
+    nwg = C.c_int32(0)
+    mode = TRAIN_SELF_COUNTS | (TRAIN_COUNT_PARTITION if count_partition else 0)
+    off = lib().objnerf_train_flat_bounds(C.byref(net), K, R, S, mode, int(bool(with_feat)), C.byref(nwg))
+    if off < 0 or nwg.value <= 0:
+        return int(nwg.value), None
+    return int(nwg.value), ws.buf[off:off + 4 * (nwg.value + 1)].view(torch.int32)
+
+
 def adamw_step(arena: ParamArena, grads: torch.Tensor, exp_avg: torch.Tensor, exp_avg_sq: torch.Tensor,
                has_grad: Optional[torch.Tensor], step: int, lr: float, weight_decay: float, beta1=0.9, beta2=0.999,
                eps=1e-8, params: Optional[torch.Tensor] = None) -> None:
```

Result: no change. 24.28 million rays/s (median of 6 runs) (+0.7%).
